# ugadiarov-la-phystech-edu/OCRL

Hardware: AMD Instinct MI355X
Metric: images/sec (node) SLATE pretrain 128x128, 6 slots, 3 iters (higher is better)
Workload: dtype f32

## Files before the change

ocrl_amd/_lib.py:

```python
import ctypes
import os
from ctypes import c_void_p

from . import _abi

_HERE = os.path.dirname(os.path.abspath(__file__))
LIB_PATH = os.environ.get("OCRL_HIP_LIB") or os.path.join(_HERE, "libocrl_hip.so")
HEADER_PATH = os.path.join(_HERE, os.pardir, "include", "ocrl_hip.h")
DQN_HEADER_PATH = os.path.join(_HERE, os.pardir, "include", "ocrl_hip_dqn.h")
ROLLOUT_HEADER_PATH = os.path.join(_HERE, os.pardir, "include", "ocrl_hip_rollout.h")
REPLAY_HEADER_PATH = os.path.join(_HERE, os.pardir, "include", "ocrl_hip_replay.h")
C51_HEADER_PATH = os.path.join(_HERE, os.pardir, "include", "ocrl_hip_c51.h")
NOISY_HEADER_PATH = os.path.join(_HERE, os.pardir, "include", "ocrl_hip_noisy.h")
CLASSIFIER_HEADER_PATH = os.path.join(_HERE, os.pardir, "include", "ocrl_hip_classifier.h")
IODINE_HEADER_PATH = os.path.join(_HERE, os.pardir, "include", "ocrl_hip_iodine.h")
QR_HEADER_PATH = os.path.join(_HERE, os.pardir, "include", "ocrl_hip_qr.h")
SLATE_KERNELS_HEADER_PATH = os.path.join(_HERE, os.pardir, "include", "ocrl_hip_slate_kernels.h")
_lib = None

if not os.path.exists(HEADER_PATH):
    raise RuntimeError(f"{HEADER_PATH} is missing: ocrl_amd derives its binding of libocrl_hip.so from the header and runs from the source tree.")
with open(HEADER_PATH) as _f:
    ABI = _abi.read(_f.read())
CONSTANTS = ABI.consts
SlateConfig, IodineConfig, GemmDesc, ConvDesc, ConvWgradDesc, XattnDesc, AcnetDesc, SpriteEnvDesc, ScenesDesc, FlatSegment = (
    ABI.structs["ocrl_" + n] for n in ("slate_config", "iodine_config", "gemm_desc", "conv_desc", "conv_wgrad_desc", "xattn_desc", "acnet_desc",
                                       "sprite_env_desc", "scenes_desc", "flat_segment"))
FLAT_MAX_SEGMENTS = CONSTANTS["OCRL_FLAT_MAX_SEGMENTS"]
if not os.path.exists(DQN_HEADER_PATH):
    raise RuntimeError(f"{DQN_HEADER_PATH} is missing: ocrl_amd derives its binding of libocrl_hip.so from the header and runs from the source tree.")
with open(DQN_HEADER_PATH) as _f:
    ABI_DQN = _abi.read(_f.read())
QnetDesc = ABI_DQN.structs["ocrl_qnet_desc"]
QNET_MAX_LAYERS = len(QnetDesc().dims)
if not os.path.exists(ROLLOUT_HEADER_PATH):
    raise RuntimeError(f"{ROLLOUT_HEADER_PATH} is missing: ocrl_amd derives its binding of libocrl_hip.so from the header and runs from the source tree.")
with open(ROLLOUT_HEADER_PATH) as _f:
    ABI_ROLLOUT = _abi.read(_f.read())
if not os.path.exists(REPLAY_HEADER_PATH):
    raise RuntimeError(f"{REPLAY_HEADER_PATH} is missing: ocrl_amd derives its binding of libocrl_hip.so from the header and runs from the source tree.")
with open(REPLAY_HEADER_PATH) as _f:
    ABI_REPLAY = _abi.read(_f.read())
if not os.path.exists(C51_HEADER_PATH):
    raise RuntimeError(f"{C51_HEADER_PATH} is missing: ocrl_amd derives its binding of libocrl_hip.so from the header and runs from the source tree.")
with open(C51_HEADER_PATH) as _f:
    ABI_C51 = _abi.read(_f.read())
C51Desc = ABI_C51.structs["ocrl_c51_desc"]
if not os.path.exists(NOISY_HEADER_PATH):
    raise RuntimeError(f"{NOISY_HEADER_PATH} is missing: ocrl_amd derives its binding of libocrl_hip.so from the header and runs from the source tree.")
with open(NOISY_HEADER_PATH) as _f:
    ABI_NOISY = _abi.read(_f.read())
NoisyDesc = ABI_NOISY.structs["ocrl_noisy_desc"]
NOISY_MAX_LAYERS = len(NoisyDesc().out)
if not os.path.exists(CLASSIFIER_HEADER_PATH):
    raise RuntimeError(f"{CLASSIFIER_HEADER_PATH} is missing: ocrl_amd derives its binding of libocrl_hip.so from the header and runs from the source tree.")
with open(CLASSIFIER_HEADER_PATH) as _f:
    ABI_CLASSIFIER = _abi.read(_f.read())
if not os.path.exists(IODINE_HEADER_PATH):
    raise RuntimeError(f"{IODINE_HEADER_PATH} is missing: ocrl_amd derives its binding of libocrl_hip.so from the header and runs from the source tree.")
with open(IODINE_HEADER_PATH) as _f:
    ABI_IODINE = _abi.read(_f.read())
if not os.path.exists(QR_HEADER_PATH):
    raise RuntimeError(f"{QR_HEADER_PATH} is missing: ocrl_amd derives its binding of libocrl_hip.so from the header and runs from the source tree.")
with open(QR_HEADER_PATH) as _f:
    ABI_QR = _abi.read(_f.read())
QrDesc = ABI_QR.structs["ocrl_qr_desc"]
if not os.path.exists(SLATE_KERNELS_HEADER_PATH):
    raise RuntimeError(f"{SLATE_KERNELS_HEADER_PATH} is missing: ocrl_amd derives its binding of libocrl_hip.so from the header and runs from the source tree.")
with open(SLATE_KERNELS_HEADER_PATH) as _f:
    ABI_SLATE_KERNELS = _abi.read(_f.read())


def flat_segments(segs):
    addr = lambda a: a.value if isinstance(a, c_void_p) else a
    return (FlatSegment * len(segs))(*[FlatSegment(addr(p), addr(g), addr(s0), addr(s1), int(n)) for p, g, s0, s1, n in segs])


def acnet_desc(B, F, A, dims, acts):
    d = AcnetDesc(B=B, F=F, A=A)
    for t in range(3):
        if len(dims[t]) > CONSTANTS["OCRL_ACNET_MAX_LAYERS"]:
            raise ValueError(f"ocrl_amd: at most {CONSTANTS['OCRL_ACNET_MAX_LAYERS']} layers per trunk (got {len(dims[t])})")
        d.n[t] = len(dims[t])
        for l, (w, a) in enumerate(zip(dims[t], acts[t])):
            d.dims[t][l], d.acts[t][l] = int(w), int(a)
    return d


def qnet_desc(B, F, A, dims, acts):
    if len(dims) > QNET_MAX_LAYERS or len(acts) != len(dims):
        raise ValueError(f"ocrl_amd: at most {QNET_MAX_LAYERS} hidden layers, one activation code each (got {len(dims)}, {len(acts)})")
    d = QnetDesc(B=B, F=F, A=A, n=len(dims))
    for l, (w, a) in enumerate(zip(dims, acts)):
        d.dims[l], d.acts[l] = int(w), int(a)
    return d


def c51_desc(B, F, A, Z, dims, acts, dueling=False):
    if len(dims) > len(C51Desc().dims) or len(acts) != len(dims):
        raise ValueError(f"ocrl_amd: at most {len(C51Desc().dims)} hidden layers, one activation code each (got {len(dims)}, {len(acts)})")
    d = C51Desc(B=B, F=F, A=A, Z=Z, n=len(dims), dueling=int(bool(dueling)))
    for l, (w, a) in enumerate(zip(dims, acts)):
        d.dims[l], d.acts[l] = int(w), int(a)
    return d


def qr_desc(B, F, A, N, dims, acts, dueling=False):
    if len(dims) > len(QrDesc().dims) or len(acts) != len(dims):
        raise ValueError(f"ocrl_amd: at most {len(QrDesc().dims)} hidden layers, one activation code each (got {len(dims)}, {len(acts)})")
    d = QrDesc(B=B, F=F, A=A, N=N, n=len(dims), dueling=int(bool(dueling)))
    for l, (w, a) in enumerate(zip(dims, acts)):
        d.dims[l], d.acts[l] = int(w), int(a)
    return d


def noisy_desc(layers):
    layers = list(layers)
    if not 1 <= len(layers) <= NOISY_MAX_LAYERS:
        raise ValueError(f"ocrl_amd: 1 .. {NOISY_MAX_LAYERS} noisy layers (got {len(layers)})")
    d = NoisyDesc(n_layers=len(layers))
    for l, (i, o) in enumerate(layers):
        getattr(d, "in")[l], d.out[l] = int(i), int(o)
    return d


def gemm_desc(**kw):
    d = GemmDesc(batch=1, batch_inner=1, splitk=1, alpha=1.0, x_scale=1.0, e_scale=1.0, force_sb=-1)
    for k, v in kw.items():
        setattr(d, k, v)
    return d


def conv_desc(**kw):
    d = ConvDesc()
    for k, v in kw.items():
        setattr(d, k, v)
    return d


def conv_wgrad_desc(**kw):
    d = ConvWgradDesc()
    for k, v in kw.items():
        setattr(d, k, v)
    return d


def lib():
    global _lib
    if _lib is not None:
        return _lib
    if not os.path.exists(LIB_PATH):
        raise RuntimeError(
            f"{LIB_PATH} is missing: build it with `python -c 'import __graft_entry__ as g; g.build()'` "
            "(make -C ocrl_amd/csrc).  ocrl_amd has no CPU fallback.")
    import torch
    L = ctypes.CDLL(LIB_PATH)
    for abi in (ABI, ABI_DQN, ABI_ROLLOUT, ABI_REPLAY, ABI_C51, ABI_NOISY, ABI_CLASSIFIER, ABI_IODINE, ABI_QR, ABI_SLATE_KERNELS):
        for name, (restype, argtypes) in abi.functions.items():
            f = getattr(L, name)
            f.argtypes = argtypes
            if restype is not ctypes.c_int:
                f.restype = restype
    for name, cls in {**ABI.structs, **ABI_DQN.structs, **ABI_C51.structs, **ABI_NOISY.structs, **ABI_QR.structs}.items():
        if name + "_size" in {**ABI.functions, **ABI_DQN.functions, **ABI_C51.functions, **ABI_NOISY.functions, **ABI_QR.functions} and getattr(L, name + "_size")() != ctypes.sizeof(cls):
            raise RuntimeError(f"libocrl_hip.so: {name} is {getattr(L, name + '_size')()} bytes, this binding's {cls.__name__} {ctypes.sizeof(cls)}")
    if L.ocrl_abi_version() != CONSTANTS["OCRL_ABI_VERSION"]:
        raise RuntimeError(f"libocrl_hip.so ABI version mismatch: the library is {L.ocrl_abi_version()}, include/ocrl_hip.h {CONSTANTS['OCRL_ABI_VERSION']}")
    _lib = L
    return L


def check(rc):
    if rc:
        raise RuntimeError("ocrl_hip: " + lib().ocrl_last_error().decode())


def ptr(t):
    return None if t is None else ctypes.c_void_p(t.data_ptr())


def ptrs(ts):
    return (ctypes.c_void_p * len(ts))(*[t.data_ptr() if t is not None else None for t in ts])


def stream(device=None):
    import torch
    return ctypes.c_void_p(torch.cuda.current_stream(device).cuda_stream)
```

ocrl_amd/csrc/elementwise.hip:

```cpp
#include "common.h"
#include "kernels.h"
#include "layernorm16.h"

#define TINYF 1.17549435e-38f

__device__ inline float block_sum(float v, float* red) {
    v = wave_sum(v);
    const int w = threadIdx.x >> 6, nw = blockDim.x >> 6;
    __syncthreads();
    if ((threadIdx.x & 63) == 0) red[w] = v;
    __syncthreads();
    float s = 0.f;
    for (int i = 0; i < nw; ++i) s += red[i];
    return s;
}
__device__ inline float block_max(float v, float* red) {
    v = wave_max(v);
    const int w = threadIdx.x >> 6, nw = blockDim.x >> 6;
    __syncthreads();
    if ((threadIdx.x & 63) == 0) red[w] = v;
    __syncthreads();
    float s = red[0];
    for (int i = 1; i < nw; ++i) s = fmaxf(s, red[i]);
    return s;
}

__global__ void nchw_to_nhwc8_kernel(const float* __restrict__ in, float* __restrict__ out, int B, int C, int H, int W) {
    const long long n = (long long)B * H * W;
    const long long i = (long long)blockIdx.x * blockDim.x + threadIdx.x;
    if (i >= n) return;
    const long long hw = (long long)H * W;
    const long long b = i / hw, r = i % hw;
    float v[8];
#pragma unroll
    for (int c = 0; c < 8; ++c) v[c] = c < C ? in[(b * C + c) * hw + r] : 0.f;
    float4* o = reinterpret_cast<float4*>(out + i * 8);
    o[0] = make_float4(v[0], v[1], v[2], v[3]);
    o[1] = make_float4(v[4], v[5], v[6], v[7]);
}

__global__ void patchify4_kernel(const float* __restrict__ in, float* __restrict__ out, int B, int C, int S) {
    const int E = S / 4;
    const long long n = (long long)B * E * E * C * 4;
    const long long i = (long long)blockIdx.x * blockDim.x + threadIdx.x;
    if (i >= n) return;
    const int ky = i & 3;
    const int c = (i >> 2) % C;
    const long long row = (i >> 2) / C;
    const int ex = row % E, ey = (row / E) % E;
    const long long b = row / ((long long)E * E);
    const float4 v = *reinterpret_cast<const float4*>(in + ((b * C + c) * S + (ey * 4 + ky)) * S + ex * 4);
    *reinterpret_cast<float4*>(out + row * (C * 16) + c * 16 + ky * 4) = v;
}

__global__ void pixel_shuffle_kernel(const float* __restrict__ in, float* __restrict__ out, int B, int h, int w, int Cout, int forward,
                                     const float* __restrict__ mask) {
    const long long n = (long long)B * h * w * Cout;
    const long long i = (long long)blockIdx.x * blockDim.x + threadIdx.x;
    if (i >= n) return;
    const int c = i % Cout;
    long long r = i / Cout;
    const int x = r % w; r /= w;
    const int y = r % h;
    const long long b = r / h;
    const long long u = i * 4;
    const long long s00 = ((b * 2 * h + 2 * y) * (2 * w) + 2 * x) * Cout + c;
    const long long s01 = s00 + Cout, s10 = s00 + (long long)2 * w * Cout, s11 = s10 + Cout;
    if (forward) {
        const float4 v = *reinterpret_cast<const float4*>(in + u);
        out[s00] = v.x; out[s01] = v.y; out[s10] = v.z; out[s11] = v.w;
    } else {
        float4 v = make_float4(in[s00], in[s01], in[s10], in[s11]);
        if (mask) {
            const float4 m = *reinterpret_cast<const float4*>(mask + u);
            v.x = m.x > 0.f ? v.x : 0.f; v.y = m.y > 0.f ? v.y : 0.f; v.z = m.z > 0.f ? v.z : 0.f; v.w = m.w > 0.f ? v.w : 0.f;
        }
        *reinterpret_cast<float4*>(out + u) = v;
    }
}

template <int NPL>
__global__ void layernorm_fwd_kernel(const float* __restrict__ x, const float* __restrict__ g, const float* __restrict__ bta,
                                     float* __restrict__ y, float* __restrict__ mean, float* __restrict__ rstd, long long R) {
    constexpr int F = 64 * NPL;
    const int lane = threadIdx.x & 63;
    const long long row = (long long)blockIdx.x * (blockDim.x >> 6) + (threadIdx.x >> 6);
    if (row >= R) return;
    float v[NPL];
    float s = 0.f;
#pragma unroll
    for (int i = 0; i < NPL; ++i) { v[i] = x[row * F + i * 64 + lane]; s += v[i]; }
    const float mu = wave_sum(s) * (1.0f / F);
    float q = 0.f;
#pragma unroll
    for (int i = 0; i < NPL; ++i) { const float d = v[i] - mu; q += d * d; }
    const float rs = rsqrtf(wave_sum(q) * (1.0f / F) + 1e-5f);
#pragma unroll
    for (int i = 0; i < NPL; ++i) {
        const int c = i * 64 + lane;
        y[row * F + c] = (v[i] - mu) * rs * g[c] + bta[c];
    }
    if (lane == 0) {
        if (mean) mean[row] = mu;
        if (rstd) rstd[row] = rs;
    }
}

template <int NPL>
__global__ void layernorm_bwd_kernel(const float* __restrict__ dy, const float* __restrict__ x, const float* __restrict__ mean,
                                     const float* __restrict__ rstd, const float* __restrict__ g, float* __restrict__ dx,
                                     float* __restrict__ part, long long R, int accumulate) {
    constexpr int F = 64 * NPL;
    __shared__ float red[4][2 * F];
    const int lane = threadIdx.x & 63, wv = threadIdx.x >> 6;
    float dg[NPL], db[NPL], gg[NPL];
#pragma unroll
    for (int i = 0; i < NPL; ++i) { dg[i] = 0.f; db[i] = 0.f; gg[i] = g[i * 64 + lane]; }
    for (long long row = (long long)blockIdx.x * 4 + wv; row < R; row += (long long)gridDim.x * 4) {
        const float mu = mean[row], rs = rstd[row];
        float xh[NPL], d[NPL];
        float s1 = 0.f, s2 = 0.f;
#pragma unroll
        for (int i = 0; i < NPL; ++i) {
            const int c = i * 64 + lane;
            xh[i] = (x[row * F + c] - mu) * rs;
            const float dyv = dy[row * F + c];
            dg[i] += dyv * xh[i];
            db[i] += dyv;
            d[i] = dyv * gg[i];
            s1 += d[i];
            s2 += d[i] * xh[i];
        }
        s1 = wave_sum(s1) * (1.0f / F);
        s2 = wave_sum(s2) * (1.0f / F);
#pragma unroll
        for (int i = 0; i < NPL; ++i) {
            const int c = i * 64 + lane;
            const float v = rs * (d[i] - s1 - xh[i] * s2);
            dx[row * F + c] = accumulate ? dx[row * F + c] + v : v;
        }
    }
#pragma unroll
    for (int i = 0; i < NPL; ++i) { red[wv][i * 64 + lane] = dg[i]; red[wv][F + i * 64 + lane] = db[i]; }
    __syncthreads();
    for (int c = threadIdx.x; c < 2 * F; c += blockDim.x)
        part[(size_t)blockIdx.x * 2 * F + c] = red[0][c] + red[1][c] + red[2][c] + red[3][c];
}

template <int NV, int NP>
__global__ __launch_bounds__(256) void layernorm16_fwd_kernel(const float* __restrict__ x, const float* __restrict__ g, const float* __restrict__ bta,
                                                              float* __restrict__ y, float* __restrict__ mean, float* __restrict__ rstd, long long R) {
    constexpr int F = 64 * NV;
    const int lane = threadIdx.x & 63, wv = threadIdx.x >> 6, c4 = lane & 15, rsub = lane >> 4;
    const long long row0 = ((long long)blockIdx.x * 4 + wv) * (4 * NP) + rsub;
    float4 v[NP][NV];
#pragma unroll
    for (int i = 0; i < NP; ++i)
#pragma unroll
        for (int k = 0; k < NV; ++k) {
            const long long row = row0 + 4 * i;
            v[i][k] = row < R ? *reinterpret_cast<const float4*>(x + row * F + (k * 16 + c4) * 4) : make_float4(0.f, 0.f, 0.f, 0.f);
        }
    float4 gg[NV], bb[NV];
#pragma unroll
    for (int k = 0; k < NV; ++k) { gg[k] = *reinterpret_cast<const float4*>(g + (k * 16 + c4) * 4); bb[k] = *reinterpret_cast<const float4*>(bta + (k * 16 + c4) * 4); }
#pragma unroll
    for (int i = 0; i < NP; ++i) {
        const long long row = row0 + 4 * i;
        float mu, rs;
        layernorm16_row_fwd<NV>(v[i], mu, rs);
        if (row < R) {
#pragma unroll
            for (int k = 0; k < NV; ++k) *reinterpret_cast<float4*>(y + row * F + (k * 16 + c4) * 4) = layernorm16_affine(v[i][k], rs, gg[k], bb[k]);
            if (c4 == 0) {
                if (mean) mean[row] = mu;
                if (rstd) rstd[row] = rs;
            }
        }
    }
}
template <int NV, int NP>
__global__ __launch_bounds__(256) void layernorm16_bwd_kernel(const float* __restrict__ dy, const float* __restrict__ x, const float* __restrict__ mean,
                                                              const float* __restrict__ rstd, const float* __restrict__ g, float* __restrict__ dx,
                                                              float* __restrict__ part, long long R, int accumulate) {
    constexpr int F = 64 * NV;
    __shared__ float4 red[2][16][16 * NV];
    const int lane = threadIdx.x & 63, wv = threadIdx.x >> 6, c4 = lane & 15, rsub = lane >> 4;
    float4 gg[NV], dg[NV], db[NV];
#pragma unroll
    for (int k = 0; k < NV; ++k) { gg[k] = *reinterpret_cast<const float4*>(g + (k * 16 + c4) * 4); dg[k] = make_float4(0.f, 0.f, 0.f, 0.f); db[k] = dg[k]; }
    for (long long grp = blockIdx.x; grp * (16 * NP) < R; grp += gridDim.x) {
        const long long row0 = (grp * 4 + wv) * (4 * NP) + rsub;
        float4 xv[NP][NV], yv[NP][NV];
        float mu[NP], rs[NP];
#pragma unroll
        for (int i = 0; i < NP; ++i) {
            const long long row = row0 + 4 * i;
            const bool ok = row < R;
#pragma unroll
            for (int k = 0; k < NV; ++k) {
                xv[i][k] = ok ? *reinterpret_cast<const float4*>(x + row * F + (k * 16 + c4) * 4) : make_float4(0.f, 0.f, 0.f, 0.f);
                yv[i][k] = ok ? *reinterpret_cast<const float4*>(dy + row * F + (k * 16 + c4) * 4) : make_float4(0.f, 0.f, 0.f, 0.f);
            }
            mu[i] = ok ? mean[row] : 0.f;
            rs[i] = ok ? rstd[row] : 0.f;
        }
#pragma unroll
        for (int i = 0; i < NP; ++i) {
            const long long row = row0 + 4 * i;
            const Ln16Bwd<NV> r = layernorm16_row_bwd<NV>(xv[i], yv[i], mu[i], rs[i], gg, dg, db);
            if (row < R) {
#pragma unroll
                for (int k = 0; k < NV; ++k) {
                    float4 o = layernorm16_row_dx(r, rs[i], k);
                    float* dp = dx + row * F + (k * 16 + c4) * 4;
                    if (accumulate) { const float4 a = *reinterpret_cast<const float4*>(dp); o.x += a.x; o.y += a.y; o.z += a.z; o.w += a.w; }
                    *reinterpret_cast<float4*>(dp) = o;
                }
            }
        }
    }
#pragma unroll
    for (int k = 0; k < NV; ++k) { red[0][wv * 4 + rsub][k * 16 + c4] = dg[k]; red[1][wv * 4 + rsub][k * 16 + c4] = db[k]; }
    __syncthreads();
    if (threadIdx.x < 32 * NV) {
        const int which = threadIdx.x / (16 * NV), c = threadIdx.x % (16 * NV);
        float4 a = red[which][0][c];
#pragma unroll
        for (int k = 1; k < 16; ++k) { const float4 t = red[which][k][c]; a.x += t.x; a.y += t.y; a.z += t.z; a.w += t.w; }
        *reinterpret_cast<float4*>(part + (size_t)blockIdx.x * (2 * F) + which * F + c * 4) = a;
    }
}

__global__ void colsum_kernel(const float* __restrict__ X, long long ld, float* __restrict__ part, long long R, int F, long long rows_per_chunk) {
    __shared__ float red[4][64];
    const int col = blockIdx.x * 64 + (threadIdx.x & 63), rl = threadIdx.x >> 6;
    const long long r0 = (long long)blockIdx.y * rows_per_chunk;
    const long long r1 = min(R, r0 + rows_per_chunk);
    float s = 0.f;
    if (col < F)
        for (long long r = r0 + rl; r < r1; r += 4) s += X[r * ld + col];
    red[rl][threadIdx.x & 63] = s;
    __syncthreads();
    if (rl == 0 && col < F) part[(size_t)blockIdx.y * F + col] = red[0][threadIdx.x] + red[1][threadIdx.x] + red[2][threadIdx.x] + red[3][threadIdx.x];
}
__global__ __launch_bounds__(256) void colsum4_kernel(const float* __restrict__ X, long long ld, float* __restrict__ part, long long R, int F,
                                                      long long rows_per_chunk) {
    __shared__ float4 red[256];
    const int F4 = F >> 2, RL = 256 / F4;
    const int c4 = threadIdx.x % F4, rl = threadIdx.x / F4;
    const long long r0 = (long long)blockIdx.x * rows_per_chunk;
    const long long r1 = min(R, r0 + rows_per_chunk);
    float4 s0 = make_float4(0.f, 0.f, 0.f, 0.f), s1 = s0, s2 = s0, s3 = s0;
    if (rl < RL) {
        const float* base = X + (size_t)c4 * 4;
        long long r = r0 + rl;
        for (; r + 3 * RL < r1; r += 4 * RL) {
            const float4 a = *reinterpret_cast<const float4*>(base + r * ld), b = *reinterpret_cast<const float4*>(base + (r + RL) * ld);
            const float4 c = *reinterpret_cast<const float4*>(base + (r + 2 * RL) * ld), d = *reinterpret_cast<const float4*>(base + (r + 3 * RL) * ld);
            s0.x += a.x; s0.y += a.y; s0.z += a.z; s0.w += a.w;
            s1.x += b.x; s1.y += b.y; s1.z += b.z; s1.w += b.w;
            s2.x += c.x; s2.y += c.y; s2.z += c.z; s2.w += c.w;
            s3.x += d.x; s3.y += d.y; s3.z += d.z; s3.w += d.w;
        }
        for (; r < r1; r += RL) {
            const float4 a = *reinterpret_cast<const float4*>(base + r * ld);
            s0.x += a.x; s0.y += a.y; s0.z += a.z; s0.w += a.w;
        }
    }
    red[threadIdx.x] = make_float4(s0.x + s1.x + s2.x + s3.x, s0.y + s1.y + s2.y + s3.y, s0.z + s1.z + s2.z + s3.z, s0.w + s1.w + s2.w + s3.w);
    __syncthreads();
    if (threadIdx.x < F4) {
        float4 t = red[threadIdx.x];
        for (int k = 1; k < RL; ++k) { const float4 v = red[k * F4 + threadIdx.x]; t.x += v.x; t.y += v.y; t.z += v.z; t.w += v.w; }
        *reinterpret_cast<float4*>(part + (size_t)blockIdx.x * F + threadIdx.x * 4) = t;
    }
}
__global__ __launch_bounds__(256) void colsum_final_kernel(const float* __restrict__ part, float* __restrict__ out, int nchunk, int F, int accumulate, float scale) {
    __shared__ float red[16][16];
    const int cl = threadIdx.x & 15, rl = threadIdx.x >> 4;
    const int c = blockIdx.x * 16 + cl;
    float s0 = 0.f, s1 = 0.f;
    if (c < F) {
        int k = rl;
        for (; k + 16 < nchunk; k += 32) { s0 += part[(size_t)k * F + c]; s1 += part[(size_t)(k + 16) * F + c]; }
        if (k < nchunk) s0 += part[(size_t)k * F + c];
    }
    red[rl][cl] = s0 + s1;
    __syncthreads();
    if (rl == 0 && c < F) {
        float t = 0.f;
#pragma unroll
        for (int k = 0; k < 16; ++k) t += red[k][cl];
        t *= scale;
        out[c] = accumulate ? out[c] + t : t;
    }
}

__global__ void reduce_partials_kernel(const float* __restrict__ part, int n, float* __restrict__ out, float scale, int accumulate) {
    __shared__ float red[4];
    float s = 0.f;
    for (int i = threadIdx.x; i < n; i += blockDim.x) s += part[i];
    s = block_sum(s, red);
    if (threadIdx.x == 0) out[0] = (accumulate ? out[0] : 0.f) + s * scale;
}

__global__ void mse_kernel(const float* __restrict__ obs, const float* __restrict__ recon, float* __restrict__ drecon,
                           float* __restrict__ part, int B, int C, int H, int W, float inv_b) {
    __shared__ float red[4];
    const long long n = (long long)B * H * W, hw = (long long)H * W;
    float s = 0.f;
    for (long long i = (long long)blockIdx.x * blockDim.x + threadIdx.x; i < n; i += (long long)gridDim.x * blockDim.x) {
        const long long b = i / hw, r = i % hw;
        const float4 rc = *reinterpret_cast<const float4*>(recon + i * 4);
        const float rv[4] = {rc.x, rc.y, rc.z, rc.w};
        float d[4] = {0.f, 0.f, 0.f, 0.f};
        for (int c = 0; c < C; ++c) {
            const float e = rv[c] - obs[(b * C + c) * hw + r];
            s += e * e;
            d[c] = 2.f * e * inv_b;
        }
        if (drecon) *reinterpret_cast<float4*>(drecon + i * 4) = make_float4(d[0], d[1], d[2], d[3]);
    }
    s = block_sum(s, red);
    if (threadIdx.x == 0) part[blockIdx.x] = s;
}

#define GS_MAXPT 16
template <int NPT>
__global__ __launch_bounds__(256) void gumbel_softmax_kernel(const float* __restrict__ raw, const float* __restrict__ e1,
                                                             const float* __restrict__ e2, float* __restrict__ z,
                                                             int* __restrict__ tokens, int V, float inv_tau,
                                                             unsigned long long seed, float* __restrict__ zst) {
    __shared__ float red[4];
    __shared__ float redv[4];
    __shared__ int redi[4];
    const long long row = blockIdx.x;
    const float* r = raw + row * V;
    const int npt = NPT ? NPT : V / 256;
    float x[GS_MAXPT];
    float mx = -INFINITY;
#pragma unroll
    for (int i = 0; i < GS_MAXPT; ++i)
        if (i < npt) { x[i] = r[i * 256 + threadIdx.x]; mx = fmaxf(mx, x[i]); }
    mx = block_max(mx, red);
    float s = 0.f;
#pragma unroll
    for (int i = 0; i < GS_MAXPT; ++i)
        if (i < npt) s += __expf(x[i] - mx);
    s = block_sum(s, red);
    const float lse = mx + __logf(s);
    float u[GS_MAXPT];
    float best = -INFINITY;
    int besti = 0;
    float m2 = -INFINITY;
#pragma unroll
    for (int i = 0; i < GS_MAXPT; ++i)
        if (i < npt) {
            const int v = i * 256 + threadIdx.x;
            const float lp = x[i] - lse;
            float ea, eb;
            if (e1) { ea = e1[row * V + v]; eb = e2[row * V + v]; }
            else {
                const uint64_t idx = (uint64_t)row * V + v;
                const uint2 ba = rng_bits4(seed, SITE_GUMBEL_Z, idx);
                ea = -__logf(u01_24(ba.x));
                eb = -__logf(u01_24(ba.y));
            }
            const float g1 = -__logf(ea + TINYF), g2 = -__logf(eb + TINYF);
            u[i] = (lp + g1) * inv_tau;
            m2 = fmaxf(m2, u[i]);
            const float h = (lp + g2) * inv_tau;
            if (h > best) { best = h; besti = v; }
        }
    m2 = block_max(m2, red);
    float s2 = 0.f;
#pragma unroll
    for (int i = 0; i < GS_MAXPT; ++i)
        if (i < npt) { u[i] = __expf(u[i] - m2); s2 += u[i]; }
    s2 = block_sum(s2, red);
    const float inv = 1.0f / s2;
#pragma unroll
    for (int i = 0; i < GS_MAXPT; ++i)
        if (i < npt) z[row * V + i * 256 + threadIdx.x] = u[i] * inv;
    if (zst) {
        float b1 = -1.f;
        int b1i = 0;
#pragma unroll
        for (int i = 0; i < GS_MAXPT; ++i)
            if (i < npt && u[i] > b1) { b1 = u[i]; b1i = i * 256 + threadIdx.x; }
        wave_argmax(b1, b1i);
        __shared__ float hv[4];
        __shared__ int hi[4];
        if ((threadIdx.x & 63) == 0) { hv[threadIdx.x >> 6] = b1; hi[threadIdx.x >> 6] = b1i; }
        __syncthreads();
        for (int k = 0; k < 4; ++k)
            if (hv[k] > b1 || (hv[k] == b1 && hi[k] < b1i)) { b1 = hv[k]; b1i = hi[k]; }
#pragma unroll
        for (int i = 0; i < GS_MAXPT; ++i)
            if (i < npt) {
                const int v = i * 256 + threadIdx.x;
                const float ys = u[i] * inv;
                zst[row * V + v] = ((v == b1i ? 1.f : 0.f) - ys) + ys;
            }
    }
    wave_argmax(best, besti);
    const int w = threadIdx.x >> 6;
    if ((threadIdx.x & 63) == 0) { redv[w] = best; redi[w] = besti; }
    __syncthreads();
    if (threadIdx.x == 0) {
        for (int k = 1; k < 4; ++k)
            if (redv[k] > best || (redv[k] == best && redi[k] < besti)) { best = redv[k]; besti = redi[k]; }
        tokens[row] = besti;
    }
}

template <int NPT>
__global__ __launch_bounds__(256) void softmax_bwd_rows_kernel(const float* __restrict__ z, float* __restrict__ d, int V, float scale) {
    __shared__ float red[4];
    const long long row = blockIdx.x;
    const int npt = NPT ? NPT : V / 256;
    float zz[GS_MAXPT], dd[GS_MAXPT];
    float s = 0.f;
#pragma unroll
    for (int i = 0; i < GS_MAXPT; ++i)
        if (i < npt) {
            zz[i] = z[row * V + i * 256 + threadIdx.x];
            dd[i] = d[row * V + i * 256 + threadIdx.x];
            s += zz[i] * dd[i];
        }
    s = block_sum(s, red);
#pragma unroll
    for (int i = 0; i < GS_MAXPT; ++i)
        if (i < npt) d[row * V + i * 256 + threadIdx.x] = zz[i] * (dd[i] - s) * scale;
}

struct CdfArgs { const float* scores; int V; float tau; unsigned long long seed; };
__device__ __forceinline__ float wave_incl_scan(float v, int lane) {
#pragma unroll
    for (int o = 1; o < 64; o <<= 1) {
        const float t = __shfl_up(v, o, 64);
        if (lane >= o) v += t;
    }
    return v;
}
__global__ __launch_bounds__(1024) void softmax_stat_combine_kernel(const float* __restrict__ stat, int nseg, long long R, float* __restrict__ lse,
                                                                    const float* __restrict__ hstat, const int* __restrict__ hidx,
                                                                    int* __restrict__ tokens, const float* __restrict__ pred, int ldp,
                                                                    const int* __restrict__ tok, float* __restrict__ part, CdfArgs cdf) {
// ... 351 lines not shown
}
__global__ void store_u64_kernel(unsigned long long* dst, unsigned long long v) { *dst = v; }
__global__ void slot_init_kernel(const float* __restrict__ mu, const float* __restrict__ logsig, const float* __restrict__ noise,
                                 float* __restrict__ slots0, long long n, int D, unsigned long long seed, const unsigned long long* __restrict__ seed_dev) {
    const long long i = (long long)blockIdx.x * blockDim.x + threadIdx.x;
    if (i >= n) return;
    if (seed_dev) seed = *seed_dev;
    const int c = i % D;
    slots0[i] = mu[c] + __expf(logsig[c]) * slot_eps(noise, i, seed);
}
__global__ __launch_bounds__(1024) void slot_init_bwd_kernel(const float* __restrict__ d, const float* __restrict__ logsig, const float* __restrict__ noise,
                                                             float* __restrict__ dmu, float* __restrict__ dlogsig, int R, int D, unsigned long long seed) {
    __shared__ float ra[16][64], rb[16][64];
    const int cl = threadIdx.x & 63, rl = threadIdx.x >> 6;
    const int c = blockIdx.x * 64 + cl;
    float a = 0.f, b = 0.f;
    if (c < D)
        for (int r = rl; r < R; r += 16) {
            const float g = d[(size_t)r * D + c];
            a += g;
            b += g * slot_eps(noise, (long long)r * D + c, seed);
        }
    ra[rl][cl] = a; rb[rl][cl] = b;
    __syncthreads();
    if (rl == 0 && c < D) {
        float sa = 0.f, sb = 0.f;
#pragma unroll
        for (int k = 0; k < 16; ++k) { sa += ra[k][cl]; sb += rb[k][cl]; }
        dmu[c] = sa;
        dlogsig[c] = sb * __expf(logsig[c]);
    }
}
__global__ void copy_kernel(const float* __restrict__ src, float* __restrict__ dst, long long n) {
    const long long i = (long long)blockIdx.x * blockDim.x + threadIdx.x;
    if (i < n) dst[i] = src[i];
}

__global__ __launch_bounds__(256) void argmax_pos_kernel(const float* __restrict__ pred, int* __restrict__ tokens, int T, int V, int t, int dense_rows) {
    __shared__ float rv[4];
    __shared__ int ri[4];
    const long long row = (long long)blockIdx.x * T + t;
    const float* r = pred + (dense_rows ? (long long)blockIdx.x : row) * V;
    float best = -INFINITY;
    int bi = 0;
    for (int v = threadIdx.x; v < V; v += 256) { const float x = r[v]; if (x > best) { best = x; bi = v; } }
    wave_argmax(best, bi);
    if ((threadIdx.x & 63) == 0) { rv[threadIdx.x >> 6] = best; ri[threadIdx.x >> 6] = bi; }
    __syncthreads();
    if (threadIdx.x == 0) {
        for (int k = 1; k < 4; ++k) if (rv[k] > best || (rv[k] == best && ri[k] < bi)) { best = rv[k]; bi = ri[k]; }
        tokens[row] = bi;
    }
}
__global__ void embed_step_kernel(const int* __restrict__ tokens, const float* __restrict__ dict, const float* __restrict__ bos,
                                  const float* __restrict__ pe, float* __restrict__ out, int B, int T, int d, int t) {
    const int i = blockIdx.x * blockDim.x + threadIdx.x;
    if (i >= B * d) return;
    const int b = i / d, c = i - b * d;
    const float* src = t == 0 ? bos : dict + (size_t)tokens[b * T + t - 1] * d;
    out[i] = src[c] + pe[(size_t)t * d + c];
}
__global__ __launch_bounds__(256) void decode_attn_kernel(const float* __restrict__ qkv, float* __restrict__ out, int T, int t, int d, int h, int ld) {
    extern __shared__ float sm[];
    const int dh = d / h, nk = t + 1, tid = threadIdx.x;
    float* sc = sm;
    float* qs = sc + ((T + 3) & ~3);
    float* red = qs + 64;
    const int b = blockIdx.x / h, hd = blockIdx.x % h;
    const float* base = qkv + (size_t)b * T * ld + hd * dh;
    const float scale = rsqrtf((float)dh);
    if (tid < dh) qs[tid] = base[(size_t)t * ld + tid] * scale;
    __syncthreads();
    float mx = -INFINITY;
    for (int j = tid; j < nk; j += 256) {
        const float* kr = base + (size_t)j * ld + d;
        float a = 0.f;
        for (int c = 0; c < dh; c += 4) {
            const float4 kv = *reinterpret_cast<const float4*>(kr + c);
            a += qs[c] * kv.x + qs[c + 1] * kv.y + qs[c + 2] * kv.z + qs[c + 3] * kv.w;
        }
        sc[j] = a;
        mx = fmaxf(mx, a);
    }
    red[tid] = mx;
    __syncthreads();
    block_tree_max<256>(red);
    mx = red[0];
    __syncthreads();
    float sum = 0.f;
    for (int j = tid; j < nk; j += 256) { const float e = __expf(sc[j] - mx); sc[j] = e; sum += e; }
    red[tid] = sum;
    __syncthreads();
    block_tree_sum<256>(red);
    const float inv = 1.0f / red[0];
    __syncthreads();
    const int nsl = 256 / dh, c = tid % dh, sl = tid / dh;
    float acc = 0.f;
    if (sl < nsl)
        for (int j = sl; j < nk; j += nsl) acc += sc[j] * base[(size_t)j * ld + 2 * d + c];
    red[tid] = sl < nsl ? acc : 0.f;
    __syncthreads();
    if (tid < dh) {
        float a = 0.f;
        for (int k = 0; k < nsl; ++k) a += red[k * dh + tid];
        out[(size_t)b * d + hd * dh + tid] = a * inv;
    }
}

__global__ void onehot_kernel(const int* __restrict__ tokens, float* __restrict__ z, long long n, int V) {
    const long long i = (long long)blockIdx.x * blockDim.x + threadIdx.x;
    if (i >= n) return;
    z[i] = (int)(i % V) == tokens[i / V] ? 1.f : 0.f;
}

int nchw_to_nhwc8_launch(const float* in, float* out, int B, int C, int H, int W, hipStream_t st) {
    OCRL_REQUIRE(C <= 8, "nchw_to_nhwc8: C must be <= 8");
    const long long n = (long long)B * H * W;
    hipLaunchKernelGGL(nchw_to_nhwc8_kernel, GRID1D(n), 0, st, in, out, B, C, H, W);
    OCRL_CHECK_LAUNCH("nchw_to_nhwc8");
    return 0;
}
int patchify4_launch(const float* in, float* out, int B, int C, int S, hipStream_t st) {
    OCRL_REQUIRE(S % 4 == 0, "patchify4: S %% 4 != 0");
    const long long n = (long long)B * (S / 4) * (S / 4) * C * 4;
    hipLaunchKernelGGL(patchify4_kernel, GRID1D(n), 0, st, in, out, B, C, S);
    OCRL_CHECK_LAUNCH("patchify4");
    return 0;
}
int pixel_shuffle_launch(const float* in, float* out, int B, int h, int w, int Cout, int forward, const float* mask, hipStream_t st) {
    const long long n = (long long)B * h * w * Cout;
    hipLaunchKernelGGL(pixel_shuffle_kernel, GRID1D(n), 0, st, in, out, B, h, w, Cout, forward, mask);
    OCRL_CHECK_LAUNCH("pixel_shuffle");
    return 0;
}
int layernorm_fwd_launch(const float* x, const float* g, const float* b, float* y, float* mean, float* rstd, long long R, int F, hipStream_t st) {
    OCRL_REQUIRE(F % 64 == 0 && F >= 64 && F <= 256, "layernorm: F must be 64..256, multiple of 64 (got %d)", F);
    dim3 grid(cdiv(R, 4)), blk(256);
    const bool al16 = aligned16(x, y, g, b);
    switch (F / 64) {
        case 1:
            if (al16) hipLaunchKernelGGL((layernorm16_fwd_kernel<1, 4>), dim3((unsigned)cdiv(R, 64)), blk, 0, st, x, g, b, y, mean, rstd, R);
            else hipLaunchKernelGGL(layernorm_fwd_kernel<1>, grid, blk, 0, st, x, g, b, y, mean, rstd, R);
            break;
        case 2: hipLaunchKernelGGL(layernorm_fwd_kernel<2>, grid, blk, 0, st, x, g, b, y, mean, rstd, R); break;
        case 3:
            if (al16) hipLaunchKernelGGL((layernorm16_fwd_kernel<3, 2>), dim3((unsigned)cdiv(R, 32)), blk, 0, st, x, g, b, y, mean, rstd, R);
            else hipLaunchKernelGGL(layernorm_fwd_kernel<3>, grid, blk, 0, st, x, g, b, y, mean, rstd, R);
            break;
        default: hipLaunchKernelGGL(layernorm_fwd_kernel<4>, grid, blk, 0, st, x, g, b, y, mean, rstd, R); break;
    }
    OCRL_CHECK_LAUNCH("layernorm_fwd");
    return 0;
}
int colsum_launch(const float* X, long long ld, float* out, long long R, int F, int accumulate, float scale, float* ws, size_t ws_floats, hipStream_t st) {
    if (F % 4 == 0 && ld % 4 == 0 && F <= 1024 && F >= 4 && (((uintptr_t)X) & 15) == 0 && R >= 1024) {
        long long nchunk = 2048;
        if (nchunk > R / 8) nchunk = R / 8;
        if ((size_t)nchunk * F > ws_floats) nchunk = (long long)(ws_floats / F);
        if (nchunk >= 16) {
            const long long rpc = (R + nchunk - 1) / nchunk;
            nchunk = (R + rpc - 1) / rpc;
            hipLaunchKernelGGL(colsum4_kernel, dim3((unsigned)nchunk), dim3(256), 0, st, X, ld, ws, R, F, rpc);
            OCRL_CHECK_LAUNCH("colsum4");
            hipLaunchKernelGGL(colsum_final_kernel, dim3(cdiv(F, 16)), dim3(256), 0, st, ws, out, (int)nchunk, F, accumulate, scale);
            OCRL_CHECK_LAUNCH("colsum_final");
            return 0;
        }
    }
    const int cb = cdiv(F, 64);
    long long nchunk = 1024 / cb;
    if (nchunk < 1) nchunk = 1;
    if (nchunk > (R + 63) / 64) nchunk = (R + 63) / 64;
    if (nchunk < 1) nchunk = 1;
    OCRL_REQUIRE((size_t)nchunk * F <= ws_floats, "colsum: workspace too small (%lld x %d)", nchunk, F);
    const long long rpc = (R + nchunk - 1) / nchunk;
    hipLaunchKernelGGL(colsum_kernel, dim3(cb, (int)nchunk), dim3(256), 0, st, X, ld, ws, R, F, rpc);
    OCRL_CHECK_LAUNCH("colsum");
    hipLaunchKernelGGL(colsum_final_kernel, dim3(cdiv(F, 16)), dim3(256), 0, st, ws, out, (int)nchunk, F, accumulate, scale);
    OCRL_CHECK_LAUNCH("colsum_final");
    return 0;
}
int layernorm_bwd_launch(const float* dy, const float* x, const float* mean, const float* rstd, const float* g, float* dx,
                         float* dgb, long long R, int F, int accumulate_dx, int accumulate_dgb, float* ws, size_t ws_floats, hipStream_t st) {
    OCRL_REQUIRE(F % 64 == 0 && F >= 64 && F <= 256, "layernorm bwd: F must be 64..256, multiple of 64 (got %d)", F);
    int nblk = (int)((R + 3) / 4);
    if (nblk > 2048) nblk = 2048;
    while (nblk > 64 && (size_t)nblk * 2 * F * 2 + (size_t)8 * 2 * F > ws_floats) nblk /= 2;
    const size_t need = (size_t)nblk * 2 * F;
    OCRL_REQUIRE(need + (size_t)8 * 2 * F <= ws_floats, "layernorm bwd: workspace too small");
    dim3 grid(nblk), blk(256);
    const bool al16 = aligned16(x, dy, dx, g, ws);
    switch (F / 64) {
        case 1:
            if (al16) hipLaunchKernelGGL((layernorm16_bwd_kernel<1, 4>), grid, blk, 0, st, dy, x, mean, rstd, g, dx, ws, R, accumulate_dx);
            else hipLaunchKernelGGL(layernorm_bwd_kernel<1>, grid, blk, 0, st, dy, x, mean, rstd, g, dx, ws, R, accumulate_dx);
            break;
        case 2: hipLaunchKernelGGL(layernorm_bwd_kernel<2>, grid, blk, 0, st, dy, x, mean, rstd, g, dx, ws, R, accumulate_dx); break;
        case 3:
            if (al16) hipLaunchKernelGGL((layernorm16_bwd_kernel<3, 2>), grid, blk, 0, st, dy, x, mean, rstd, g, dx, ws, R, accumulate_dx);
            else hipLaunchKernelGGL(layernorm_bwd_kernel<3>, grid, blk, 0, st, dy, x, mean, rstd, g, dx, ws, R, accumulate_dx);
            break;
        default: hipLaunchKernelGGL(layernorm_bwd_kernel<4>, grid, blk, 0, st, dy, x, mean, rstd, g, dx, ws, R, accumulate_dx); break;
    }
    OCRL_CHECK_LAUNCH("layernorm_bwd");
    return colsum_launch(ws, 2 * F, dgb, nblk, 2 * F, accumulate_dgb, 1.f, ws + need, ws_floats - need, st);
}
int reduce_partials_launch(const float* part, int n, float* out, float scale, int accumulate, hipStream_t st) {
    hipLaunchKernelGGL(reduce_partials_kernel, dim3(1), dim3(256), 0, st, part, n, out, scale, accumulate);
    OCRL_CHECK_LAUNCH("reduce_partials");
    return 0;
}
int mse_launch(const float* obs, const float* recon, float* drecon, float* out, int B, int C, int H, int W, float* ws, size_t ws_floats, hipStream_t st) {
    OCRL_REQUIRE(C <= 4, "mse: C must be <= 4");
    const int nblk = 1024;
    OCRL_REQUIRE(ws_floats >= (size_t)nblk, "mse: workspace too small");
    hipLaunchKernelGGL(mse_kernel, dim3(nblk), dim3(256), 0, st, obs, recon, drecon, ws, B, C, H, W, 1.0f / B);
    OCRL_CHECK_LAUNCH("mse");
    return reduce_partials_launch(ws, nblk, out, 1.0f / B, 0, st);
}
int gumbel_softmax_launch(const float* raw, const float* e1, const float* e2, float* z, int* tokens, long long R, int V, float tau,
                          unsigned long long seed, hipStream_t st, float* zst) {
    OCRL_REQUIRE(V % 256 == 0 && V <= 256 * GS_MAXPT, "gumbel_softmax: V must be a multiple of 256, <= %d", 256 * GS_MAXPT);
    OCRL_REQUIRE((e1 == nullptr) == (e2 == nullptr), "gumbel_softmax: give both noise tensors or none");
    switch (V / 256) {
        case 16: hipLaunchKernelGGL(gumbel_softmax_kernel<16>, dim3((unsigned)R), dim3(256), 0, st, raw, e1, e2, z, tokens, V, 1.0f / tau, seed, zst); break;
        case 8: hipLaunchKernelGGL(gumbel_softmax_kernel<8>, dim3((unsigned)R), dim3(256), 0, st, raw, e1, e2, z, tokens, V, 1.0f / tau, seed, zst); break;
        default: hipLaunchKernelGGL(gumbel_softmax_kernel<0>, dim3((unsigned)R), dim3(256), 0, st, raw, e1, e2, z, tokens, V, 1.0f / tau, seed, zst); break;
    }
    OCRL_CHECK_LAUNCH("gumbel_softmax");
    return 0;
}
int softmax_bwd_rows_launch(const float* z, float* d, long long R, int V, float scale, hipStream_t st) {
    OCRL_REQUIRE(V % 256 == 0 && V <= 256 * GS_MAXPT, "softmax_bwd_rows: V must be a multiple of 256, <= %d", 256 * GS_MAXPT);
    if (V == 4096) hipLaunchKernelGGL(softmax_bwd_rows_kernel<16>, dim3((unsigned)R), dim3(256), 0, st, z, d, V, scale);
    else hipLaunchKernelGGL(softmax_bwd_rows_kernel<0>, dim3((unsigned)R), dim3(256), 0, st, z, d, V, scale);
    OCRL_CHECK_LAUNCH("softmax_bwd_rows");
    return 0;
}
int softmax_stat_combine_launch(const float* stat, int nseg, long long R, float* lse, const float* hstat, const int* hidx, int* tokens,
                                const float* pred, int ldp, const int* tok, float* out, float scale, float* ws, size_t ws_floats, hipStream_t st,
                                const float* cdf_scores, int cdf_V, float cdf_tau, unsigned long long cdf_seed) {
    OCRL_REQUIRE(nseg >= 1 && nseg <= 64, "softmax_stat_combine: 1..64 segments (got %d)", nseg);
    const long long nblk = (R + 15) / 16;
    OCRL_REQUIRE(!pred || (tok && out && ws && ws_floats >= (size_t)nblk), "softmax_stat_combine: cross-entropy needs tokens, an output and %lld workspace floats", nblk);
    CdfArgs cdf;
    cdf.scores = cdf_scores; cdf.V = cdf_V; cdf.tau = cdf_tau; cdf.seed = cdf_seed;
    OCRL_REQUIRE(!cdf_scores || (hstat && hidx && tokens && cdf_V > 0 && cdf_V <= nseg * 64), "softmax_stat_combine: inverse-CDF sampling arguments");
    hipLaunchKernelGGL(softmax_stat_combine_kernel, dim3((unsigned)nblk), dim3(1024), 0, st, stat, nseg, R, lse, hstat, hidx, tokens, pred, ldp, tok,
                       pred ? ws : nullptr, cdf);
    OCRL_CHECK_LAUNCH("softmax_stat_combine");
    if (pred) return reduce_partials_launch(ws, (int)nblk, out, scale, 0, st);
    return 0;
}
int exp_rows_launch(const float* y, const float* lse, float* z, long long R, int V, hipStream_t st) {
    OCRL_REQUIRE(V % 4 == 0, "exp_rows: V %% 4 != 0");
    const long long n4 = R * (V / 4);
    hipLaunchKernelGGL(exp_rows_kernel, dim3((unsigned)((n4 + 255) / 256)), dim3(256), 0, st, y, lse, z, n4, V / 4);
    OCRL_CHECK_LAUNCH("exp_rows");
    return 0;
}
int rowdot_bias64_launch(const float* g, const float* act, const float* bias, long long R, float* out, hipStream_t st) {
    OCRL_REQUIRE(((((uintptr_t)g) | ((uintptr_t)act) | ((uintptr_t)bias)) & 15) == 0, "rowdot: operands must be 16-byte aligned");
    hipLaunchKernelGGL(rowdot_bias64_kernel, dim3((unsigned)((R + 15) / 16)), dim3(256), 0, st, g, act, bias, R, out);
    OCRL_CHECK_LAUNCH("rowdot_bias64");
    return 0;
}
int embed_fwd_launch(const int* tokens, const float* dict, const float* bos, const float* pe, float* out, int B, int T, int d, float p,
                     unsigned long long seed, hipStream_t st) {
    OCRL_REQUIRE(d % 4 == 0, "embed: d %% 4 != 0");
    const long long n = (long long)B * T * (d / 4);
    hipLaunchKernelGGL(embed_fwd_kernel, dim3((unsigned)cdiv(n, 1024)), dim3(256), 0, st, tokens, dict, bos, pe, out, B, T, d, p, seed);
    OCRL_CHECK_LAUNCH("embed_fwd");
    return 0;
}
static size_t eb_align(size_t n) { return (n + 63) & ~(size_t)63; }
size_t embed_bwd_ws_floats(long long BT, int V, int d) {
    const size_t nchunk = (size_t)cdiv(BT, EB_CHUNK), nunit = (size_t)cdiv(BT, EB_UNIT);
    return eb_align(nchunk * (V + 1)) + 2 * eb_align((size_t)V + 2) + eb_align((size_t)BT) + eb_align(nunit * 2 * d);
}
int embed_bwd_launch(float* g, const int* tokens, float* ddict, int B, int T, int V, int d, float p, unsigned long long seed, float* ws,
                     size_t ws_floats, hipStream_t st) {
    const long long BT = (long long)B * T;
    OCRL_REQUIRE(d % 4 == 0 && d <= 1024 && V + 1 <= 16384 && BT < (1ll << 31), "embed_bwd: unsupported shape (d %d, vocabulary %d, %lld rows)", d, V, BT);
    OCRL_REQUIRE(ws && ws_floats >= embed_bwd_ws_floats(BT, V, d), "embed_bwd: scratch too small");
    const int nchunk = cdiv(BT, EB_CHUNK), nunit = cdiv(BT, EB_UNIT);
    int* hist = reinterpret_cast<int*>(ws);
    int* total = hist + eb_align((size_t)nchunk * (V + 1));
    int* base = total + eb_align((size_t)V + 2);
    int* perm = base + eb_align((size_t)V + 2);
    float* part = reinterpret_cast<float*>(perm + eb_align((size_t)BT));
    if (p > 0.f) {
        hipLaunchKernelGGL(embed_drop_bwd_kernel, GRID1D(BT * (d / 4)), 0, st, g, B, T, d, p, seed);
        OCRL_CHECK_LAUNCH("embed_drop_bwd");
    }
    hipLaunchKernelGGL(eb_hist_kernel, dim3(nchunk), dim3(256), (V + 1) * sizeof(int), st, tokens, hist, BT, T, V);
    hipLaunchKernelGGL(eb_scan_chunks_kernel, dim3(cdiv(V + 1, 256)), dim3(256), 0, st, hist, total, nchunk, V);
    hipLaunchKernelGGL(eb_base_kernel, dim3(1), dim3(1024), 0, st, total, base, V);
    hipLaunchKernelGGL(eb_place_kernel, dim3(nchunk), dim3(256), 0, st, tokens, hist, base, perm, BT, T, V);
    const int nthr = (d + 63) & ~63;
    hipLaunchKernelGGL(eb_segsum_kernel, dim3(nunit), dim3(nthr), 0, st, g, tokens, perm, base, total, ddict, part, BT, T, V, d);
    hipLaunchKernelGGL(eb_combine_kernel, dim3(V), dim3(nthr), 0, st, base, total, part, ddict, V, d);
    OCRL_CHECK_LAUNCH("embed_bwd");
    return 0;
}
int dropout_apply_launch(const float* x, float* y, long long n, float p, unsigned long long seed, unsigned site, hipStream_t st) {
    OCRL_REQUIRE(n % 4 == 0, "dropout_apply: n %% 4 != 0");
    hipLaunchKernelGGL(dropout_apply_kernel, GRID1D(n / 4), 0, st, x, y, n / 4, p, seed, site);
    OCRL_CHECK_LAUNCH("dropout_apply");
    return 0;
}
int dropout_mask_launch(float* y, long long n, float p, unsigned long long seed, unsigned site, hipStream_t st) {
    hipLaunchKernelGGL(dropout_mask_kernel, GRID1D(n), 0, st, y, n, p, seed, site);
    OCRL_CHECK_LAUNCH("dropout_mask");
    return 0;
}
__global__ void obs_u8_to_f32_kernel(const unsigned char* __restrict__ in, float* __restrict__ out, long long npix_total, long long HW, int C) {
    const long long i = (long long)blockIdx.x * blockDim.x + threadIdx.x;
    if (i >= npix_total) return;
    const long long b = i / HW, pix = i - b * HW;
    const unsigned char* src = in + i * C;
    float* dst = out + b * C * HW + pix;
    for (int c = 0; c < C; ++c) dst[c * HW] = (float)src[c] / 255.0f;
}
int obs_u8_to_f32_launch(const unsigned char* in, float* out, int B, int H, int W, int C, hipStream_t st) {
    const long long n = (long long)B * H * W;
    hipLaunchKernelGGL(obs_u8_to_f32_kernel, GRID1D(n), 0, st, in, out, n, (long long)H * W, C);
    OCRL_CHECK_LAUNCH("obs_u8_to_f32");
    return 0;
}
int fill_launch(float* x, long long n, float v, hipStream_t st) {
    hipLaunchKernelGGL(fill_kernel, GRID1D(n), 0, st, x, n, v);
    OCRL_CHECK_LAUNCH("fill");
    return 0;
}
int axpy_launch(const float* x, float* y, long long n, float a, hipStream_t st) {
    hipLaunchKernelGGL(axpy_kernel, GRID1D(n), 0, st, x, y, n, a);
    OCRL_CHECK_LAUNCH("axpy");
    return 0;
}
int posmap_launch(const float* Wpos, const float* bpos, float* out, int S, int C, hipStream_t st) {
    hipLaunchKernelGGL(posmap_kernel, GRID1D((long long)S * S * C), 0, st, Wpos, bpos, out, S, C);
    OCRL_CHECK_LAUNCH("posmap");
    return 0;
}
int posgrid_launch(float* out, int S, hipStream_t st) {
    hipLaunchKernelGGL(posgrid_kernel, GRID1D(S * S), 0, st, out, S);
    OCRL_CHECK_LAUNCH("posgrid");
    return 0;
}
int pad_cols_launch(const float* in, int ldi, float* out, int ldo, long long R, int C, int Cout, hipStream_t st) {
    hipLaunchKernelGGL(pad_cols_kernel, GRID1D(R * Cout), 0, st, in, ldi, out, ldo, R, C, Cout);
    OCRL_CHECK_LAUNCH("pad_cols");
    return 0;
}
int store_u64_launch(unsigned long long* dst, unsigned long long v, hipStream_t st) {
    hipLaunchKernelGGL(store_u64_kernel, dim3(1), dim3(1), 0, st, dst, v);
    OCRL_CHECK_LAUNCH("store_u64");
    return 0;
// ... 57 lines not shown
```

ocrl_amd/csrc/kernels.h:

```cpp
#pragma once
#include "common.h"
#include "../../include/ocrl_hip.h"

enum { PROF_CONV5 = 0, PROF_CONV_OTHER = 1, PROF_WGRAD = 2, PROF_GEMM = 3, PROF_SA_FWD = 4, PROF_SA_BWD = 5, PROF_ATTN_FWD = 6, PROF_ATTN_BWD = 7, PROF_NTAGS = 8 };
int prof_begin(int tag, hipStream_t st);
void prof_end(int idx, hipStream_t st);

struct GemmArgs {
    const float* A = nullptr;
    const float* B = nullptr;
    float* C = nullptr;
    int M = 0, N = 0, K = 0;
    int lda = 0, ldb = 0, ldc = 0;
    int akc = 1, bkc = 1;
    int batch = 1;
    int batch_inner = 1;
    long long sA = 0, sB = 0, sC = 0;
    long long sAi = 0, sBi = 0, sCi = 0;
    int splitk = 1;
    long long sCsplit = 0;
    float alpha = 1.f;
    const float* bias = nullptr;
    int relu = 0;
    float drop_p = 0.f;
// ... 60 lines not shown
    float p = 0.f; unsigned long long seed = 0; unsigned site = 0;
};
int pool_cls_attn_fwd_launch(const PoolClsArgs& a, hipStream_t st);
int pool_cls_attn_bwd_launch(const PoolClsArgs& a, hipStream_t st);
int pool_flash_launch(const float* qkv, float* O, float* lse, const float* dO, float* Dd, float* dqkv, int B, int S, int d, int h, float p,
                      unsigned long long seed, unsigned site, int backward, hipStream_t st);

int rn_pair_fwd_launch(const float* AB, const float* b1, float* h1, int B, int K, int g, hipStream_t st);
int rn_pair_bwd_launch(const float* dh1, float* dAB, int B, int K, int g, hipStream_t st);
int rn_pairsum_fwd_launch(const float* gL, float* y, int B, int P, int g, hipStream_t st);
int rn_pairsum_bwd_launch(const float* dy, const float* gL, float* dgL, int B, int P, int g, hipStream_t st);

struct NcMap { long long sN = 0, sG = 0, sC = 0, sH = 0, sW = 0; };
struct NcFwdArgs {
    const float* X = nullptr; NcMap x;
    float* Y = nullptr; float* Y2 = nullptr; NcMap y;
    const float* w[OCRL_NATURECNN_MAX_GROUPS] = {}; const float* bias[OCRL_NATURECNN_MAX_GROUPS] = {};
    int B = 0, G = 1, cin = 0, cout = 0, H = 0, W = 0, OH = 0, OW = 0, ks = 0, stride = 0;
    int pad = 0;
};
struct NcBwdArgs {
    const float* X = nullptr; NcMap x;
    const float* dY = nullptr; NcMap dy;
    float* dX = nullptr;
    float* part = nullptr;
    int slabs = 1, slab_rows = 0;
    const float* w[OCRL_NATURECNN_MAX_GROUPS] = {};
    int B = 0, G = 1, cin = 0, cout = 0, H = 0, W = 0, OH = 0, OW = 0, ks = 0, stride = 0;
    int pad = 0;
    long long dw_tiles = 0, dx_tiles = 0; int dw_blocks = 0;
};
struct NcReduceLayer { const float* part = nullptr; int slabs = 0, G = 0, cout = 0, K = 0; long long n = 0; };
struct NcReduceArgs {
    NcReduceLayer L[OCRL_NATURECNN_MAX_CONVS];
    float* dw[OCRL_NATURECNN_MAX_CONVS][OCRL_NATURECNN_MAX_GROUPS] = {};
    float* db[OCRL_NATURECNN_MAX_CONVS][OCRL_NATURECNN_MAX_GROUPS] = {};
    int nlayers = 0;
};
int nc_conv_fwd_launch(const NcFwdArgs& a, hipStream_t st);
int nc_conv_bwd_launch(NcBwdArgs a, hipStream_t st);
int nc_dw_reduce_launch(const NcReduceArgs& a, hipStream_t st);
int nc_relu_mask_launch(const float* d, const float* act, float* out, long long n, hipStream_t st);

struct PcGeom {
    int OH = 0, OW = 0, OWT = 0;
    int NG = 0, nchunk = 0;
    size_t wp_floats = 0;
    long long units = 0; int slab_units = 0, slabs = 0; size_t part_floats = 0;
    int passes = 0, nbg = 0, Dp = 0; size_t wd_floats = 0;
    int HB = 0, WB = 0, WT = 0; long long dx_units = 0; int upw = 0;
};
PcGeom pc_geom(int B, int H, int W, int D);
struct PcFwdArgs {
    const float* X = nullptr; const float* Wp = nullptr; const float* bias = nullptr; float* Y = nullptr;
    int B = 0, H = 0, W = 0, D = 0, OH = 0, OW = 0, OWT = 0, nchunk = 0, NG = 0;
};
struct PcDwArgs {
    const float* X = nullptr; const float* dY = nullptr; float* part = nullptr; float* partb = nullptr;
    int B = 0, H = 0, W = 0, D = 0, OH = 0, OW = 0, OWT = 0, nchunk = 0, slab_units = 0;
    long long units = 0;
};
struct PcDxArgs {
    const float* dY = nullptr; const float* Wd = nullptr; float* dX = nullptr;
    int H = 0, W = 0, D = 0, OH = 0, OW = 0, HB = 0, WT = 0, Dp = 0, passes = 0, upw = 0;
    long long units = 0, groups = 0;
};
int pc_conv1_fwd_launch(const float* X, const float* w, const float* bias, float* Wp, float* Y, int B, int H, int W, int D, hipStream_t st);
int pc_conv1_dw_launch(const float* X, const float* dY, float* part, int B, int H, int W, int D, hipStream_t st);
int pc_conv1_dw_reduce_launch(const float* part, float* dw, float* db, int B, int H, int W, int D, hipStream_t st);
int pc_conv1_dx_launch(const float* dY, const float* w, float* Wd, float* dX, int B, int H, int W, int D, hipStream_t st);

#define PROBE_MAX_SLOTS 12
#define PROBE_MAX_PROPS 8
#define PROBE_MAX_WIDTH 256
struct ProbeSchema { int P; int t[PROBE_MAX_PROPS], a[PROBE_MAX_PROPS], b[PROBE_MAX_PROPS], kind[PROBE_MAX_PROPS]; };
int probe_schema_check(const ProbeSchema& sc, int T, int O);
int probe_match_check(int B, int K, int N, int T, int O);
int probe_match_launch(const float* out, int ld_row, long long ld_img, const float* y, const float* dloss, float* cost, int* col, float* part,
                       float* metrics, float* dout, int B, int K, int N, int T, int O, const ProbeSchema& sc, hipStream_t st);
int probe_leaky_fwd_launch(float* x, long long n, float slope, hipStream_t st);
int probe_leaky_bwd_launch(float* dx, const float* h, long long n, float slope, hipStream_t st);

int vae_permute_launch(const float* src, float* dst, long long R, int C, int HW, int rows, int pack, hipStream_t st);
int vae_pad_rows_launch(const float* src, float* dst, int rows, int rows_pad, int K, hipStream_t st);
int vae_kl_fwd_launch(const float* ml, const float* eps, float* latent, float* part, float* rep, int B, int L, hipStream_t st);
int vae_loss_launch(const float* part, float* metrics, int B, float kld_weight, hipStream_t st);
int vae_kl_bwd_launch(const float* ml, const float* eps, const float* dlat, const float* drep, const float* dloss, float* dml, int B, int L,
                      float kld_weight, hipStream_t st);
int vae_scale_launch(const float* x, float* y, const float* g, long long n, hipStream_t st);
int vae_recon_nchw_launch(const float* r4, float* out, int B, int C, int HW, hipStream_t st);

#define MAE_MAX_PATCHES 1024
int mae_rank_launch(const float* noise, int* restore, int* keep, float* mask, int* restore_out, float* mask_out, int B, int L, int len_keep,
                    hipStream_t st);
int mae_patch_gather_launch(const float* obs, const int* ids, float* out, int B, int n, int S, int p, hipStream_t st);
int mae_tokens_fwd_launch(const float* embed, const float* cls, const float* pos, const int* ids, float* x0, int B, int n, int D, hipStream_t st);
int mae_tokens_bwd_launch(const float* dx0, float* dembed, float* dcls, int B, int n, int D, hipStream_t st);
int mae_unshuffle_fwd_launch(const float* e, const float* mtok, const float* dpos, const int* restore, float* xd, int B, int L, int len_keep, int Dd,
                             hipStream_t st);
int mae_unshuffle_bwd_launch(const float* dxd, const int* keep, const float* mask, float* de, float* dmtok, float* part, int B, int L, int len_keep,
                             int Dd, hipStream_t st);
int mae_gelu_fwd_launch(const float* pre, float* y, long long n, hipStream_t st);
int mae_gelu_bwd_launch(const float* dy, const float* pre, float* dpre, long long n, hipStream_t st);
int mae_ln_fwd_launch(const float* x, const float* g, const float* b, float* y, float* mean, float* rstd, long long R, int F, float eps, hipStream_t st);
int mae_ln_chunks(long long R);
int mae_ln_bwd_launch(const float* dy, const float* x, const float* mean, const float* rstd, const float* g, const float* resid, float* dx, float* dg,
                      float* db, float* part, long long R, int F, hipStream_t st);
int mae_loss_launch(const float* pred, const float* obs, const float* mask, const float* dloss, float* part, float* loss, float* dpred, int B, int L,
                    int len_keep, int S, int p, hipStream_t st);

struct ConvArgs {
    const float* X = nullptr;
    const float* Wp = nullptr;
    float* Y = nullptr;
    int B = 0, H = 0, W = 0;
    const float* bias = nullptr;
    int relu = 0;
    const float* posmap = nullptr;
    const float* mask = nullptr;
    int mask_elu = 0;
};
size_t conv_x3_pack_floats(int KS = 5);
int conv_pack_x3_launch(const float* W, float* fwd3, float* bwd3, hipStream_t st, int KS = 5);
int conv_x3_launch(const ConvArgs& a, const float* pack3, hipStream_t st, int KS = 5);
struct WgradArgs;
int conv_wgrad_x3_stage(const WgradArgs& a, int nchunk, hipStream_t st, int KS = 5);
struct WgradArgs {
    const float* X = nullptr;
    const float* dY = nullptr;
    float* part = nullptr;
    int B = 0, H = 0, W = 0;
    float* bpart = nullptr;
};
int conv_fwd_launch(const ConvArgs& a, int KS, int CIN, int COUT, hipStream_t st, int low_latency = 0);
int conv_wgrad_launch(const WgradArgs& a, int KS, int CIN, int COUT, int cin_real, float* dW, float* db, int accumulate, hipStream_t st, int x3 = -1);
int conv_wgrad_slabs(int B, int H, int W, int KS, int CIN);
size_t conv_wgrad_ws_floats(int B, int H, int W, int KS, int CIN, bool with_db = true);
int conv_pack_launch(const float* W, float* fwd, float* bwd, int KS, int CIN, int COUT, int cin_real, hipStream_t st);

size_t conv_first_pack_floats();
int conv_first_pack_launch(const float* W, float* pack, hipStream_t st);
int conv_first_fwd_launch(const float* obs, const float* pack, const float* bias, float* Y, int B, int H, int W, int relu, hipStream_t st);
int conv_first_wgrad_workers(int B, int H, int W);
size_t conv_first_wgrad_ws_floats(int B, int H, int W);
int conv_first_wgrad_launch(const float* obs, const float* dY, float* ws, float* dW, float* db, int B, int H, int W, int accumulate, hipStream_t st);

int nchw_to_nhwc8_launch(const float* in, float* out, int B, int C, int H, int W, hipStream_t st);
int patchify4_launch(const float* in, float* out, int B, int C, int S, hipStream_t st);
int pixel_shuffle_launch(const float* in, float* out, int B, int h, int w, int Cout, int forward, const float* mask, hipStream_t st);
int layernorm_fwd_launch(const float* x, const float* g, const float* b, float* y, float* mean, float* rstd, long long R, int F, hipStream_t st);
int layernorm_bwd_launch(const float* dy, const float* x, const float* mean, const float* rstd, const float* g, float* dx,
                         float* dgb, long long R, int F, int accumulate_dx, int accumulate_dgb, float* ws, size_t ws_floats, hipStream_t st);
int colsum_launch(const float* X, long long ld, float* out, long long R, int F, int accumulate, float scale, float* ws, size_t ws_floats, hipStream_t st);

#define SA_INPUT_SLAB (2 * 4096 + 4 * 64)
void sa_input_plan(long long R, int max_wgs, int out[3]);
int sa_input_fwd_launch(const float* e4, const float* gamma, const float* beta, const float* W0, const float* b0, const float* W2, const float* b2,
                        float* mean, float* rstd, float* ln0, float* h1, float* x, long long R, int max_wgs, hipStream_t st);
int sa_input_bwd_launch(const float* dx, const float* h1, const float* e4, const float* mean, const float* rstd, const float* gamma, const float* beta,
                        const float* W0, const float* W2, float* de4, float* dW0, float* db0, float* dW2, float* db2, float* dgamma, float* dbeta,
                        long long R, int max_wgs, float* ws, size_t ws_floats, hipStream_t st);
int reduce_partials_launch(const float* part, int n, float* out, float scale, int accumulate, hipStream_t st);
int mse_launch(const float* obs, const float* recon, float* drecon, float* out, int B, int C, int H, int W, float* ws, size_t ws_floats, hipStream_t st);
int gumbel_softmax_launch(const float* raw, const float* e1, const float* e2, float* z, int* tokens, long long R, int V, float tau,
                          unsigned long long seed, hipStream_t st, float* zst = nullptr);
int softmax_bwd_rows_launch(const float* z, float* d, long long R, int V, float scale, hipStream_t st);
int softmax_stat_combine_launch(const float* stat, int nseg, long long R, float* lse, const float* hstat, const int* hidx, int* tokens,
                                const float* pred, int ldp, const int* tok, float* out, float scale, float* ws, size_t ws_floats, hipStream_t st,
                                const float* cdf_scores = nullptr, int cdf_V = 0, float cdf_tau = 1.f, unsigned long long cdf_seed = 0);
int exp_rows_launch(const float* y, const float* lse, float* z, long long R, int V, hipStream_t st);
int rowdot_bias64_launch(const float* g, const float* act, const float* bias, long long R, float* out, hipStream_t st);
int embed_fwd_launch(const int* tokens, const float* dict, const float* bos, const float* pe, float* out, int B, int T, int d, float p,
                     unsigned long long seed, hipStream_t st);
size_t embed_bwd_ws_floats(long long BT, int V, int d);
int embed_bwd_launch(float* g, const int* tokens, float* ddict, int B, int T, int V, int d, float p, unsigned long long seed, float* ws,
                     size_t ws_floats, hipStream_t st);
int dropout_apply_launch(const float* x, float* y, long long n, float p, unsigned long long seed, unsigned site, hipStream_t st);
int dropout_mask_launch(float* y, long long n, float p, unsigned long long seed, unsigned site, hipStream_t st);
int obs_u8_to_f32_launch(const unsigned char* in, float* out, int B, int H, int W, int C, hipStream_t st);
int fill_launch(float* x, long long n, float v, hipStream_t st);
int axpy_launch(const float* x, float* y, long long n, float a, hipStream_t st);
int posmap_launch(const float* Wpos, const float* bpos, float* out, int S, int C, hipStream_t st);
int posgrid_launch(float* out, int S, hipStream_t st);
int im2col5_launch(const float* x8, float* col, long long npix, int H, int W, int C, int ldc, hipStream_t st);
int unpack5_launch(const float* dWp, float* dW, int C, int ldc, hipStream_t st);
int pad_cols_launch(const float* in, int ldi, float* out, int ldo, long long R, int C, int Cout, hipStream_t st);

struct XaPlan { bool supported = false; int KP = 0, NC = 0, NM = 0; size_t lds = 0; };
bool xattn_plan(int K, int d, int h, XaPlan* out);
bool xattn_supported(int K, int d, int h);
int xattn_kp(int K, int h);
struct XaFoldHost {
    const float* mem = nullptr;
    const float* Wq[8]; const float* Wk[8]; const float* Wv[8]; const float* Wo[8];
    float* ck[8]; float* cv[8];
    float* Ab[8]; float* AbT[8]; float* Vo[8]; float* VoT[8];
    int B = 0, K = 0, d = 0, h = 0, nblk = 0;
};
int xattn_fold_fwd_launch(const XaFoldHost& f, hipStream_t st);
struct XaHost {
    const float* x = nullptr;
    const float* resid = nullptr;
    float* y = nullptr;
    float* P = nullptr;
    const float *Ab = nullptr, *AbT = nullptr, *Vo = nullptr, *VoT = nullptr;
    const float* gd = nullptr;
    float *Pd = nullptr, *dS = nullptr;
    int B = 0, T = 0, K = 0, d = 0, h = 0;
    float p = 0.f; unsigned long long seed = 0; unsigned site_p = 0, site_o = 0;
};
int xattn_launch(const XaHost& h, int backward, hipStream_t st);
struct XaFoldBwdHost {
    const float *Pd = nullptr, *dS = nullptr;
    const float *gd = nullptr, *x = nullptr;
    const float *Wq = nullptr, *Wo = nullptr;
    const float *ck = nullptr, *cv = nullptr;
    float *dVo = nullptr, *dAb = nullptr;
    float *dck = nullptr, *dcv = nullptr;
    float *pq = nullptr, *po = nullptr;
    float *dWq = nullptr, *dWo = nullptr;
    float* ws = nullptr; size_t ws_floats = 0;
    int B = 0, T = 0, K = 0, d = 0, h = 0;
};
int xattn_fold_bwd_launch(const XaFoldBwdHost& f, hipStream_t st);
int cross_attn_fwd_launch(const float* Q, const float* Km, const float* Vm, float* O, float* P, int B, int T, int K, int d, int h, float p,
                          unsigned long long seed, unsigned site, hipStream_t st);
size_t cross_attn_bwd_ws_floats(int B, int T, int K, int d, int h);
int cross_attn_bwd_launch(const float* dO, const float* Q, const float* Km, const float* Vm, const float* P, float* dQ, float* dKm, float* dVm,
                          int B, int T, int K, int d, int h, float p, unsigned long long seed, unsigned site, float* part, size_t part_floats,
                          hipStream_t st);


struct SaWts {
    int ln_in_g, ln_in_b, ln_s_g, ln_s_b, ln_m_g, ln_m_b;
    int Wq, WqT, Wk, WkT, Wv, WvT, Wih, WihT, Whh, WhhT, bih, bhh, W0, W0T, b0, W2, W2T, b2;
    int total;
};
static inline SaWts sa_wts_layout(int C, int D, int H) {
    SaWts o; int a = 0;
    auto take = [&](int n) { int r = a; a += (n + 3) & ~3; return r; };
    o.ln_in_g = take(C); o.ln_in_b = take(C); o.ln_s_g = take(D); o.ln_s_b = take(D); o.ln_m_g = take(D); o.ln_m_b = take(D);
    o.Wq = take(D * D); o.WqT = take(D * D); o.Wk = take(D * C); o.WkT = take(C * D); o.Wv = take(D * C); o.WvT = take(C * D);
    o.Wih = take(3 * D * D); o.WihT = take(3 * D * D); o.Whh = take(3 * D * D); o.WhhT = take(3 * D * D);
    o.bih = take(3 * D); o.bhh = take(3 * D);
    o.W0 = take(H * D); o.W0T = take(H * D); o.b0 = take(H); o.W2 = take(D * H); o.W2T = take(D * H); o.b2 = take(D);
    o.total = a;
    return o;
}
struct SaSave { int sprev, sn, q, u, r, z, n, hn, sg, m, hid, qp, up, upn, csum, ld; };
static inline SaSave sa_save_layout(int C, int D, int H, int NH = 1) {
    SaSave o;
    o.sprev = 0; o.sn = D; o.q = 2 * D; o.u = 3 * D; o.r = 4 * D; o.z = 5 * D; o.n = 6 * D; o.hn = 7 * D; o.sg = 8 * D; o.m = 9 * D;
    o.hid = 10 * D; o.qp = 10 * D + H; o.up = o.qp + NH * C; o.upn = o.up + NH * C; o.csum = o.upn + NH * C; o.ld = o.csum + ((NH + 3) & ~3);
    return o;
}
struct SaGrad { int out, hid, gi, gh, u, q, qp, ld; };
static inline SaGrad sa_grad_layout(int C, int D, int H, int NH = 1) {
    SaGrad o;
    o.out = 0; o.hid = D; o.gi = D + H; o.gh = 4 * D + H; o.u = 7 * D + H; o.q = 8 * D + H; o.qp = 9 * D + H; o.ld = 9 * D + H + NH * C;
    return o;
}
struct SlotAttnArgs {
    int B = 0, N = 0, C = 64, K = 0, D = 0, H = 0, I = 0;
    int NH = 1;
    float eps = 1e-8f, scale = 1.f;
    const float* x = nullptr;
    const float* slots0 = nullptr;
    const float* wts = nullptr;
    float* slots = nullptr;
    float* attn = nullptr;
    float* attn_heads = nullptr;
    float* save = nullptr;
    const float* dslots = nullptr;
    float* dx = nullptr;
    float* dslots0 = nullptr;
    float* grows = nullptr;
    float* g_small = nullptr;
    float* xchg = nullptr;
    float* parts = nullptr;
    int phase = 0;
};
size_t sa_xchg_floats_host(int K, int D);
size_t sa_parts_floats_host(int B, int K);
struct SaPlan { int G, NB, KB, KS; size_t smem_fwd, smem_bwd; };
int sa_plan(int K, int D, int H, int NH, SaPlan* plan);
int slot_attn_launch(const SlotAttnArgs& a, int backward, hipStream_t st);

struct PackEntry { const float* src; int rows, cols, dst_off, transpose; };
int pack_launch(const PackEntry* entries_dev, int n_entries, int max_elems, float* dst, hipStream_t st);

int absmax_launch(const float* g, long long n, float* out, float* ws, size_t ws_floats, hipStream_t st);
int clip_adam_launch(float* p, const float* g, float* m, float* v, long long n, const float* norm, float clip, float lr, double b1,
                     double b2, double eps, int step, float gscale, hipStream_t st);
int clip_adam_tail_launch(float* p, const float* g, float* m, float* v, int n, const float* norm, float clip, float lr, double b1, double b2,
                          double eps, int step, float gscale, hipStream_t st);
int clip_rmsprop_launch(float* p, const float* g, float* sq, long long n, const float* norm, float clip, float lr, double alpha, double eps,
                        hipStream_t st);
int clip_rmsprop_tail_launch(float* p, const float* g, float* sq, int n, const float* norm, float clip, float lr, double alpha, double eps,
                             hipStream_t st);
constexpr int FLAT_MAX_SEG = 8, FLAT_SEG_BLOCKS = 1024;
struct FlatSegs {
    float* p[FLAT_MAX_SEG];
    const float* g[FLAT_MAX_SEG];
    float* s0[FLAT_MAX_SEG];
    float* s1[FLAT_MAX_SEG];
    long long n[FLAT_MAX_SEG];
// ... 82 lines not shown
```

ocrl_amd/csrc/slate_model.cpp:

```cpp
#include "slate_model.h"

#include "switches.h"

#include <math.h>
#include <stdarg.h>
#include <string.h>

static std::string fmt(const char* f, ...) {
    char buf[256];
    va_list ap;
    va_start(ap, f);
    vsnprintf(buf, sizeof buf, f, ap);
    va_end(ap);
    return buf;
}

SlateModel::SlateModel(const SlateConfig& c) : cfg(c) {
    S = c.obs_size; E = S / 4; T = E * E; N = S * S; V = c.vocab; d = c.d_model; C = c.cnn_hidden;
    K = c.num_slots; I = c.num_iters; D = c.slot_size; H = c.mlp_hidden; NB = c.num_blocks; NH = c.num_heads;
    DH = d / NH; Bmax = c.max_batch; SH = c.slot_heads > 0 ? c.slot_heads : 1;
    const int ch = c.obs_channels;
    add_param("_dvae._encoder.0.m.weight", {64, ch, 4, 4}, 0); add_param("_dvae._encoder.0.m.bias", {64}, 0);
    for (int i = 1; i < 7; ++i) { add_param(fmt("_dvae._encoder.%d.m.weight", i), {64, 64, 1, 1}, 0); add_param(fmt("_dvae._encoder.%d.m.bias", i), {64}, 0); }
    add_param("_dvae._encoder.7.weight", {V, 64, 1, 1}, 0); add_param("_dvae._encoder.7.bias", {V}, 0);
// ... 84 lines not shown
    for (const ParamInfo& q : params_)
        if (q.group == 1 && (q.name.rfind("_slotproj.", 0) == 0 || q.name.rfind("_dec.", 0) == 0) && q.offset < w.enc_grads_end) w.enc_grads_end = q.offset;
}

SlateModel::~SlateModel() {
    if (ev_fork_) (void)hipEventDestroy(ev_fork_);
    if (ev_join_) (void)hipEventDestroy(ev_join_);
    if (ev_tokens_) (void)hipEventDestroy(ev_tokens_);
    if (side_) (void)hipStreamDestroy(side_);
    for (auto& kv : enc_graphs_) if (kv.second.exec) (void)hipGraphExecDestroy(kv.second.exec);
    for (hipEvent_t e : ev_dw_) if (e) (void)hipEventDestroy(e);
    if (ev_join2_) (void)hipEventDestroy(ev_join2_);
    if (side2_) (void)hipStreamDestroy(side2_);
    if (cap_) (void)hipStreamDestroy(cap_);
}

void SlateModel::layout_workspace(bool commit) {
    begin_layout(commit);
    x3_of_.clear();
    const size_t B = Bmax, BT = B * T, BN = B * N, BK = B * K;
    metrics_ = carve("metrics", 64);
    scratch_floats_ = 0;
    {
        size_t need = conv_wgrad_ws_floats((int)(B * (cfg.use_bcdec ? K : 1)), S, S, 5, 64) + (size_t)512 * 2304 * 2;
        if (conv_first_wgrad_ws_floats((int)B, S, S) > need) need = conv_first_wgrad_ws_floats((int)B, S, S);
        size_t sk = (size_t)32 * V * d + (size_t)(1 << 20);
        if (sk > need) need = sk;
        size_t cs = (size_t)N * C * 8 + (size_t)T * d * 8 + (1 << 20);
        if (cs > need) need = cs;
        if (cfg.use_bcdec && bcast_l1_bwd_ws_floats((long long)BK, S, 5) > need) need = bcast_l1_bwd_ws_floats((long long)BK, S, 5);
        const size_t ca = cross_attn_bwd_ws_floats((int)B, T, K, d, NH), eb = embed_bwd_ws_floats((long long)B * T, V, d);
        if (ca > need) need = ca;
        if (eb > need) need = eb;
        scratch_floats_ = need + (1 << 20);
    }
    scratch_ = carve(nullptr, scratch_floats_);
    scratch2_ = cfg.use_bcdec ? scratch_ : carve(nullptr, scratch_floats_);
    obs8_ = first_direct() ? nullptr : carve("obs8", BN * 8);
    obs_keep_ = first_direct() ? carve(nullptr, BN * cfg.obs_channels) : nullptr;
    obs_stage_ = carve(nullptr, (B < 32 ? B : 32) * (size_t)cfg.obs_channels * N);
    seed_dev_ = reinterpret_cast<unsigned long long*>(carve(nullptr, 64));
    e1_ = carve("enc1", BN * 64); e2_ = carve("enc2", BN * 64); e3_ = carve("enc3", BN * 64); e4_ = carve("feats", BN * 64);
    posmap_ = carve(nullptr, (size_t)N * C); gridT_ = carve(nullptr, (size_t)N * 4);
    ln0_ = carve(nullptr, BN * 64); ln0_mean_ = carve(nullptr, BN); ln0_rstd_ = carve(nullptr, BN);
    h1_ = carve("sa_mlp_hidden", BN * 64); x_ = carve("sa_inputs", BN * 64);
    slots0_ = carve("slots0", BK * D); slot_noise_ = carve(nullptr, BK * D); slots_ = carve("slots", BK * D);
    attn_ = carve("attn", BN * K);
    attn_heads_ = SH > 1 ? carve(nullptr, sa_attn_heads_floats(B, N, K, SH)) : nullptr;
    const SaSizes sz = sa_sizes(B, K, C, D, H, I, SH);
    sa_save_ = carve("sa_save", sz.save);
    sa_grows_ = carve(nullptr, sz.grows);
    sa_wts_ = carve(nullptr, sz.wts);
    sa_small_ = carve(nullptr, sz.small);
    sa_xchg_ = carve(nullptr, sz.xchg);
    sa_parts_ = carve(nullptr, sz.parts);
    sa_pack_dev_ = reinterpret_cast<PackEntry*>(carve(nullptr, sz.table));
    for (int i = 0; i < 4; ++i) {
        const int cin = i == 0 ? 8 : 64;
        cw_fwd_[i] = carve(nullptr, (size_t)25 * cin * 64);
        cw_bwd_[i] = i == 0 ? nullptr : carve(nullptr, (size_t)25 * 64 * 64);
        if (conv_x3_ && i > 0) {
            float* f3 = carve(nullptr, conv_x3_pack_floats());
            float* b3 = carve(nullptr, conv_x3_pack_floats());
            if (ws_commit_) { x3_of_[cw_fwd_[i]] = f3; x3_of_[cw_bwd_[i]] = b3; }
        }
    }
    gslots_ = carve(nullptr, BK * D); gslots0_ = carve(nullptr, BK * D);
    gA_ = carve(nullptr, BN * 64); gB_ = carve(nullptr, BN * 64); gC_ = cfg.use_bcdec ? gA_ : carve(nullptr, BN * 64);
    gmap_ = carve(nullptr, (size_t)N * C);
    if (cfg.use_bcdec) {
        const size_t BKN = BK * (size_t)N;
        bc_Wc_ = carve(nullptr, 25 * 64 * 5 + 64); bc_W1r_ = carve(nullptr, (size_t)25 * 64 * D); bc_P1_ = carve(nullptr, (size_t)N * 64);
        bc_M_ = carve(nullptr, BK * 1600); bc_T_ = carve(nullptr, BK * 1600);
        bc_c1_ = carve("bc_c1", BKN * 64); bc_c2_ = carve("bc_c2", BKN * 64); bc_c3_ = carve("bc_c3", BKN * 64);
        bc_out4_ = carve(nullptr, BKN * 4); bc_dout4_ = carve(nullptr, BKN * 4);
        bc_gA_ = carve(nullptr, BKN * 64); bc_gB_ = carve(nullptr, BKN * 64);
        for (int i = 0; i < 2; ++i) {
            bc_pk_[i] = carve(nullptr, 25 * 64 * 64); bc_pkb_[i] = carve(nullptr, 25 * 64 * 64);
            if (conv_x3_ > 0) {
                float* f3 = carve(nullptr, conv_x3_pack_floats());
                float* b3 = carve(nullptr, conv_x3_pack_floats());
                if (ws_commit_) { x3_of_[bc_pk_[i]] = f3; x3_of_[bc_pkb_[i]] = b3; }
            }
        }
        bc_Wk4_ = carve(nullptr, 9 * 64 * 4); bc_Wb4_ = carve(nullptr, 9 * 64 * 4);
        bc_dW1r_ = carve(nullptr, (size_t)25 * 64 * D); bc_dWc_ = carve(nullptr, 25 * 64 * 5 + 64);
        bc_dT_ = carve(nullptr, BK * 1600); bc_dM_ = carve(nullptr, BK * 1600); bc_G1_ = carve(nullptr, (size_t)N * 64);
        recon_ = carve("recon", BN * 4);
    } else {
    patches_ = carve("patches", BT * 16 * cfg.obs_channels);
    for (int i = 0; i < 7; ++i) de_[i] = carve(fmt("dvae_enc%d", i).c_str(), BT * 64);
    zraw_ = carve("zraw", BT * V);
    z_ = carve("z", BT * V);
    zdec_ = cfg.hard ? carve("z_st", BT * V) : z_;
    tokens_ = reinterpret_cast<int*>(carve("tokens", BT));
    {
        const size_t nseg = (size_t)gemm_stat_segments(V);
        zstat_ = carve(nullptr, BT * nseg * 2); zhstat_ = carve(nullptr, BT * nseg); zhidx_ = reinterpret_cast<int*>(carve(nullptr, BT * nseg));
        zlse_ = carve("z_lse", BT); zdot_ = carve(nullptr, BT);
        cestat_ = carve(nullptr, BT * nseg * 2); celse_ = carve("ce_lse", BT); cepart_ = carve(nullptr, BT / 16 + 16);
    }
    dd0_ = carve("dvae_dec0", BT * 64); dd1_ = carve("dvae_dec1", BT * 64); dd2_ = carve("dvae_dec2", BT * 64); dd3_ = carve("dvae_dec3", BT * 64);
    dd4_ = carve("dvae_dec4", BT * 256); ps1_ = carve(nullptr, BT * 256);
    dd6_ = carve("dvae_dec6", BT * 256); dd7_ = carve("dvae_dec7", BT * 256); dd8_ = carve("dvae_dec8", BT * 256);
    dd9_ = carve("dvae_dec9", BT * 1024); ps2_ = carve(nullptr, BN * 64);
    recon_ = carve("recon", BN * 4); drecon_ = carve(nullptr, BN * 4);
    for (int i = 0; i < 2; ++i) {
        dw_fwd_[i] = carve(nullptr, 9 * 64 * 64); dw_bwd_[i] = carve(nullptr, 9 * 64 * 64);
        if (conv_x3_ > 0) {
            float* f3 = carve(nullptr, conv_x3_pack_floats(3));
            float* b3 = carve(nullptr, conv_x3_pack_floats(3));
            if (ws_commit_) { x3_of_[dw_fwd_[i]] = f3; x3_of_[dw_bwd_[i]] = b3; }
        }
    }
    w11p_ = carve(nullptr, 4 * 64);
    mem_ = carve("mem", BK * d); emb_ = carve("emb", BT * d);
    for (int b = 0; b < NB; ++b) {
        Blk& k = blk_[b];
        k.ln1 = carve(nullptr, BT * d); k.ln1_mean = carve(nullptr, BT); k.ln1_rstd = carve(nullptr, BT);
        k.q = carve(nullptr, BT * 3 * d); k.k = k.q + d; k.v = k.q + 2 * d;
        k.lse = carve(nullptr, B * NH * (size_t)T); k.ao = carve(nullptr, BT * d); k.x1 = carve(nullptr, BT * d);
        k.ln2 = carve(nullptr, BT * d); k.ln2_mean = carve(nullptr, BT); k.ln2_rstd = carve(nullptr, BT);
        k.cq = carve(nullptr, BT * d); k.ck = carve(nullptr, BK * d); k.cv = carve(nullptr, BK * d);
        k.cP = carve(nullptr, B * NH * (size_t)T * K); k.cao = carve(nullptr, BT * d); k.x2 = carve(nullptr, BT * d);
        k.ln3 = carve(nullptr, BT * d); k.ln3_mean = carve(nullptr, BT); k.ln3_rstd = carve(nullptr, BT);
        k.f1 = carve(fmt("blk%d.ffn_hidden", b).c_str(), BT * 4 * d); k.x3 = carve(nullptr, BT * d);
    }
    bg_.resize(NB);
    {
        const size_t NC = xattn_supported(K, d, NH) ? (size_t)NH * xattn_kp(K, NH) : 16;
        xa_zero_base_ = carve_pos();
        for (int b = 0; b < NB; ++b) {
            Blk& k = blk_[b];
            k.xaAb = carve(nullptr, B * NC * d); k.xaAbT = carve(nullptr, B * NC * d); k.xaVo = carve(nullptr, B * NC * d); k.xaVoT = carve(nullptr, B * NC * d);
        }
        xa_zero_floats_ = (size_t)(carve_pos() - xa_zero_base_);
        for (int b = 0; b < NB; ++b) { bg_[b].xaPd = carve(nullptr, BT * NC); bg_[b].xaDs = carve(nullptr, BT * NC); }
        xa_dAb_ = carve(nullptr, B * NC * d); xa_dVo_ = carve(nullptr, B * NC * d);
        xa_pq_ = carve(nullptr, B * (size_t)d * d); xa_po_ = carve(nullptr, B * (size_t)d * d);
    }
    attn_delta_ = carve(nullptr, B * NH * (size_t)T);
    attn_ds_ = attn_ds_floats_ ? carve(nullptr, attn_ds_floats_) : nullptr;
    lnf_ =carve("dec_out", BT * d); lnf_mean_ = carve(nullptr, BT); lnf_rstd_ = carve(nullptr, BT);
    pred_ = carve("pred", BT * V);
    gx_ = carve(nullptr, BT * d); gbr_ = carve(nullptr, BT * d); gt1_ = carve(nullptr, BT * d); gt2_ = carve(nullptr, BT * d);
    gt3_ = carve(nullptr, BT * d); gf1_ = carve(nullptr, BT * 4 * d); gqkv_ = carve(nullptr, BT * 3 * d);
    for (int b = 0; b < NB; ++b) {
        BlkG& q = bg_[b];
        if (b == 0) { q.gbr[0] = gbr_; q.gf1 = gf1_; q.gt2 = gt2_; q.gqkv = gqkv_; }
        else { q.gbr[0] = carve(nullptr, BT * d); q.gf1 = carve(nullptr, BT * 4 * d); q.gt2 = carve(nullptr, BT * d); q.gqkv = carve(nullptr, BT * 3 * d); }
        q.gbr[1] = carve(nullptr, BT * d); q.gbr[2] = carve(nullptr, BT * d);
    }
    scratch3_ = carve(nullptr, scratch_floats_);
    gmem_ = carve(nullptr, BK * d); gck_ = carve(nullptr, BK * d); gcv_ = carve(nullptr, BK * d);
    gdA_ = carve(nullptr, BN * 64); gdB_ = carve(nullptr, BN * 64);
    }
    col0_ = dw0p_ = nullptr;
    if (!first_direct()) {
        const int ldc0 = (25 * cfg.obs_channels + 3) & ~3;
        col0_ = carve(nullptr, BN * ldc0); dw0p_ = carve(nullptr, (size_t)64 * ldc0);
    }
    end_layout();
}

int SlateModel::bind(float* p, float* g, float* m, float* v, void* ws, size_t ws_bytes) {
    RC(check_buffers(p, g, ws, ws_bytes));
    OCRL_REQUIRE(d % 64 == 0 && d <= 256 && D % 64 == 0 && C == 64 && V % 256 == 0 && S % 4 == 0 && d % NH == 0 && DH % 4 == 0 && DH <= 64,
                 "unsupported configuration (d_model/slot_size multiples of 64 <= 256, cnn hidden 64, vocab %% 256, obs_size %% 4)");
    OCRL_REQUIRE(cfg.obs_channels == 3, "obs_channels must be 3");
    OCRL_REQUIRE(T % 4 == 0, "obs_size/4 squared must be a multiple of 4");
    adopt_buffers(p, g, m, v, ws);
    clear_encode_graphs();
    packs_valid_ = false;
    layout_workspace(true);
    if (!side_) {
        plan_ = stream_plan((int)sw::model<sw::OCRL_OVERLAP>(), (int)sw::model<sw::OCRL_DW_SIDE>(), sw::model<sw::OCRL_TOKENS_LATE>() != 0, cfg.use_bcdec);
        if (plan_.side) {
            OCRL_HIP(hipStreamCreateWithFlags(&side_, hipStreamNonBlocking));
            OCRL_HIP(hipEventCreateWithFlags(&ev_fork_, hipEventDisableTiming));
            OCRL_HIP(hipEventCreateWithFlags(&ev_join_, hipEventDisableTiming));
            OCRL_HIP(hipEventCreateWithFlags(&ev_tokens_, hipEventDisableTiming));
            if (plan_.dw) {
                for (hipEvent_t& ev : ev_dw_) OCRL_HIP(hipEventCreateWithFlags(&ev, hipEventDisableTiming));
                OCRL_HIP(hipEventCreateWithFlags(&ev_join2_, hipEventDisableTiming));
                if (plan_.dw == 2) OCRL_HIP(hipStreamCreateWithFlags(&side2_, hipStreamNonBlocking));
            }
        }
    }
    sa_input_ = (int)sw::model<sw::OCRL_SA_INPUT>();
    xattn_ = !cfg.use_bcdec && xattn_supported(K, d, NH) && sw::model<sw::OCRL_XATTN>() != 0;
    if (!cfg.use_bcdec && xa_zero_floats_) OCRL_HIP(hipMemset(xa_zero_base_, 0, xa_zero_floats_ * sizeof(float)));
    RC(posgrid_launch(gridT_, S, 0));
    RC(fill_launch(recon_, (long long)Bmax * N * 4, 0.f, 0));
    const float* saw[SA_NW];
    for (int i = 0; i < SA_NW; ++i) saw[i] = P(w_.sa.w[i]);
    PackEntry ent[SA_PACK_ENTRIES];
    sa_pack_n_ = sa_pack_table(saw, C, D, H, ent, &sa_pack_max_);
    OCRL_HIP(hipMemcpy(sa_pack_dev_, ent, sa_pack_n_ * sizeof(PackEntry), hipMemcpyHostToDevice));
    OCRL_HIP(hipDeviceSynchronize());
    have_fwd_ = false;
    return 0;
}

int SlateModel::soft_z(hipStream_t st) {
    if (!fused_heads() || cfg.use_bcdec) return 0;
    OCRL_REQUIRE(have_scores_, "soft_z: no forward since the last backward (the scores have been overwritten by their gradient)");
    return exp_rows_launch(zraw_, zlse_, z_, (long long)last_.B * T, V, st);
}
int SlateModel::dropout_mask(unsigned site, long long n, float* out, hipStream_t st) const {
    return dropout_mask_launch(out, n, pdrop_, last_.seed, site, st);
}

int SlateModel::conv_layer_fwd(const float* x, const float* pack, const float* bias, float* y, int Bn, int Hh, int Ww, int KS, int CIN,
                               int relu, const float* posmap, const float* mask, const Lane& L) {
    ConvArgs a;
    a.X = x; a.Wp = pack; a.Y = y; a.B = Bn; a.H = Hh; a.W = Ww; a.bias = bias; a.relu = relu; a.posmap = posmap; a.mask = mask;
    if (conv_x3_ > 0 && (KS == 5 || KS == 3) && CIN == 64 && !conv_lowlat_) {
        auto it = x3_of_.find(pack);
        if (it != x3_of_.end()) return conv_x3_launch(a, it->second, L, KS);
    }
    return conv_fwd_launch(a, KS, CIN, 64, L, conv_lowlat_);
}
int SlateModel::conv_layer_wgrad(const float* x, const float* dy, float* dW, float* db, int Bn, int Hh, int Ww, int KS, int CIN,
                                 int cin_real, const Lane& L) {
    WgradArgs a;
    a.X = x; a.dY = dy; a.part = L.scratch; a.B = Bn; a.H = Hh; a.W = Ww;
    OCRL_REQUIRE(conv_wgrad_ws_floats(Bn, Hh, Ww, KS, CIN) <= L.scratch_floats, "conv wgrad: scratch too small");
    const bool x3 = conv_x3_ > 0 && CIN == 64;
    RC(conv_wgrad_launch(a, KS, CIN, 64, cin_real, dW, x3 ? nullptr : db, 0, L, x3 ? 1 : 0));
    if (db && x3) RC(colsum_launch(dy, 64, db, (long long)Bn * Hh * Ww, 64, 0, 1.f, L.scratch, L.scratch_floats, L));
    return 0;
}

int SlateModel::pack_weights(const Lane& L, bool encoder_only) {
    if (first_direct()) RC(conv_first_pack_launch(P(w_.enc[0].w), cw_fwd_[0], L));
    else RC(conv_pack_launch(P(w_.enc[0].w), cw_fwd_[0], nullptr, 5, 8, 64, cfg.obs_channels, L));
    RC(conv_pack_launch(P(w_.enc[1].w), cw_fwd_[1], cw_bwd_[1], 5, 64, 64, 64, L));
    RC(conv_pack_launch(P(w_.enc[2].w), cw_fwd_[2], cw_bwd_[2], 5, 64, 64, 64, L));
    RC(conv_pack_launch(P(w_.enc[3].w), cw_fwd_[3], cw_bwd_[3], 5, 64, 64, 64, L));
    if (conv_x3_ > 0) {
        for (int i = 1; i < 4; ++i) {
            auto f = x3_of_.find(cw_fwd_[i]), b = x3_of_.find(cw_bwd_[i]);
            if (f != x3_of_.end()) RC(conv_pack_x3_launch(P(w_.enc[i].w), const_cast<float*>(f->second), b != x3_of_.end() ? const_cast<float*>(b->second) : nullptr, L));
        }
    }
    if (!cfg.use_bcdec && !encoder_only) {
        RC(conv_pack_launch(P(w_.dvae_dec[1].w), dw_fwd_[0], dw_bwd_[0], 3, 64, 64, 64, L));
        RC(conv_pack_launch(P(w_.dvae_dec[6].w), dw_fwd_[1], dw_bwd_[1], 3, 64, 64, 64, L));
        if (conv_x3_ > 0) {
            for (int i = 0; i < 2; ++i) {
                auto f = x3_of_.find(dw_fwd_[i]), b = x3_of_.find(dw_bwd_[i]);
                if (f != x3_of_.end()) RC(conv_pack_x3_launch(P(w_.dvae_dec[i ? 6 : 1].w), const_cast<float*>(f->second), b != x3_of_.end() ? const_cast<float*>(b->second) : nullptr, L, 3));
            }
        }
        RC(copy_launch(P(w_.dvae_dec[11].w), w11p_, cfg.obs_channels * 64, L));
        RC(fill_launch(w11p_ + cfg.obs_channels * 64, (4 - cfg.obs_channels) * 64, 0.f, L));
    }
    RC(pack_launch(sa_pack_dev_, sa_pack_n_, sa_pack_max_, sa_wts_, L));
    RC(posmap_launch(P(w_.enc_pos.w), P(w_.enc_pos.b), posmap_, S, C, L));
    return 0;
}

int SlateModel::fwd_encoder(const StepInputs& in, const Lane& L, FwdDvae fork) {
    const int B = in.B;
    const long long BN = (long long)B * N;
    auto fork_if = [&](FwdDvae here) -> int {
        if (fork != here) return 0;
        RC(after(dvae_lane(), L, ev_fork_));
        return fwd_dvae(in, dvae_lane());
    };
    RC(slot_init_launch(P(w_.sa.mu), P(w_.sa.log_sigma), in.noise_slots, slots0_, B * K, D, in.seed, L, in.seed_dev));
    SlotAttnArgs a = sa_args(B, N, K, D, H, I, SH);
    a.x = x_; a.slots0 = slots0_; a.wts = sa_wts_; a.slots = slots_; a.attn = attn_; a.attn_heads = attn_heads_; a.save = sa_save_;
    if (conv_lowlat_ && frozen_) a.save = nullptr;
    a.xchg = sa_xchg_; a.parts = sa_parts_;
    a.phase = 1;
    RC(slot_attn_launch(a, 0, L));
    RC(fork_if(FwdDvae::AtStart));
    if (first_direct()) {
        RC(conv_first_fwd_launch(in.obs, cw_fwd_[0], P(w_.enc[0].b), e1_, B, S, S, 1, L));
        if (!(conv_lowlat_ && frozen_))
            OCRL_HIP(hipMemcpyAsync(obs_keep_, in.obs, (size_t)BN * cfg.obs_channels * sizeof(float), hipMemcpyDeviceToDevice, L));
    } else {
        RC(nchw_to_nhwc8_launch(in.obs, obs8_, B, cfg.obs_channels, S, S, L));
        RC(conv_layer_fwd(obs8_, cw_fwd_[0], P(w_.enc[0].b), e1_, B, S, S, 5, 8, 1, nullptr, nullptr, L));
    }
    RC(conv_layer_fwd(e1_, cw_fwd_[1], P(w_.enc[1].b), e2_, B, S, S, 5, 64, 1, nullptr, nullptr, L));
    RC(conv_layer_fwd(e2_, cw_fwd_[2], P(w_.enc[2].b), e3_, B, S, S, 5, 64, 1, nullptr, nullptr, L));
    RC(conv_layer_fwd(e3_, cw_fwd_[3], P(w_.enc[3].b), e4_, B, S, S, 5, 64, 0, posmap_, nullptr, L));
    RC(fork_if(FwdDvae::AfterConvs));
    if (sa_input_ && C == 64 && !(conv_lowlat_ && frozen_)) {
        RC(sa_input_fwd_launch(e4_, P(w_.sa.ln.w), P(w_.sa.ln.b), P(w_.sa.mlp0.w),
                               P(w_.sa.mlp0.b), P(w_.sa.mlp2.w), P(w_.sa.mlp2.b), ln0_mean_, ln0_rstd_,
                               sa_input_ == 2 ? ln0_ : nullptr, h1_, x_, BN, 0, L));
    } else {
        RC(layernorm_fwd_launch(e4_, P(w_.sa.ln.w), P(w_.sa.ln.b), ln0_, ln0_mean_, ln0_rstd_, BN, C, L));
        RC(lin_fwd(ln0_, C, P(w_.sa.mlp0.w), P(w_.sa.mlp0.b), h1_, C, BN, C, C, 1, nullptr, 0, 0.f, 0, L));
        RC(lin_fwd(h1_, C, P(w_.sa.mlp2.w), P(w_.sa.mlp2.b), x_, C, BN, C, C, 0, nullptr, 0, 0.f, 0, L));
    }
    RC(fork_if(FwdDvae::AtSlotAttention));
    a.phase = 2;
    RC(slot_attn_launch(a, 0, L));
    return 0;
}

int SlateModel::fwd_dvae(const StepInputs& in, const Lane& L) {
// ... 132 lines not shown
    OCRL_REQUIRE(p_ && ws_, "forward: model not bound");
    OCRL_REQUIRE(in.B >= 1 && in.B <= Bmax, "forward: batch %d outside [1,%d]", in.B, Bmax);
    OCRL_REQUIRE(in.obs && in.tau > 0.f, "forward: bad inputs");
    last_ = in;
    have_enc_ = false;
    pdrop_ = in.train ? cfg.dropout : 0.f;
    const Lane L = main_lane(st);
    RC(pack_weights(L));
    if (cfg.use_bcdec) {
        RC(fwd_encoder(in, L));
        RC(pack_bcdec(L));
        RC(fwd_bcdec(L));
        RC(fill_launch(metrics_ + 1, 1, 0.f, L));
        RC(copy_launch(metrics_ + 0, metrics_ + 2, 1, L));
        have_fwd_ = true;
        return 0;
    }
    if (plan_.fwd_dvae == FwdDvae::Serial) RC(fwd_dvae(in, L));
    if (plan_.fwd_dvae == FwdDvae::BesideEncoder) {
        RC(after(dvae_lane(), L, ev_fork_));
        RC(fwd_dvae(in, dvae_lane()));
    }
    RC(fwd_encoder(in, L, plan_.fwd_dvae));
    if (plan_.tokens_early) OCRL_HIP(hipStreamWaitEvent(L, ev_tokens_, 0));
    else if (plan_.side) RC(after(L, dvae_lane(), ev_join_));
    RC(fwd_decoder(L));
    if (plan_.tokens_early) RC(after(L, dvae_lane(), ev_join_));
    RC(copy_launch(metrics_ + 0, metrics_ + 2, 1, L));
    RC(axpy_launch(metrics_ + 1, metrics_ + 2, 1, 1.f, L));
    have_fwd_ = true;
    return 0;
}

int SlateModel::encode(const StepInputs& in, hipStream_t st) {
    OCRL_REQUIRE(p_ && ws_, "encode: model not bound");
    OCRL_REQUIRE(in.B >= 1 && in.B <= Bmax && in.obs, "encode: bad inputs");
    last_ = in;
    pdrop_ = 0.f;
    have_fwd_ = false;
    have_enc_ = true;
    const Lane L = main_lane(st);
    if (enc_graph_mode_ < 0) enc_graph_mode_ = (int)sw::model<sw::OCRL_ENCODE_GRAPH>();
    const bool graph = enc_graph_mode_ && in.B <= 32 && !in.noise_slots && obs_stage_;
    const bool need_pack = !(frozen_ && packs_valid_);
    struct LowLat { int& f; LowLat(int& x) : f(x) { f = 1; } ~LowLat() { f = 0; } } lowlat(conv_lowlat_);
    if (!graph) {
        if (need_pack) RC(pack_weights(L, true));
        packs_valid_ = frozen_;
        return fwd_encoder(in, L);
    }
    EncGraph& eg = enc_graphs_[in.B];
    if (!eg.warm || need_pack) {
        eg.warm = 1;
        if (need_pack) RC(pack_weights(L, true));
        packs_valid_ = frozen_;
        return fwd_encoder(in, L);
    }
    const size_t bytes = (size_t)in.B * cfg.obs_channels * N * sizeof(float);
    OCRL_HIP(hipMemcpyAsync(obs_stage_, in.obs, bytes, hipMemcpyDeviceToDevice, L));
    RC(store_u64_launch(seed_dev_, in.seed, L));
    if (!eg.exec) {
        StepInputs gi = in;
        gi.obs = obs_stage_; gi.seed_dev = seed_dev_;
        hipGraph_t g = nullptr;
        if (!cap_) OCRL_HIP(hipStreamCreateWithFlags(&cap_, hipStreamNonBlocking));
        OCRL_HIP(hipStreamBeginCapture(cap_, hipStreamCaptureModeThreadLocal));
        const Lane cap = main_lane(cap_);
        int rc = frozen_ ? 0 : pack_weights(cap, true);
        if (!rc) rc = fwd_encoder(gi, cap);
        const hipError_t ce = hipStreamEndCapture(cap_, &g);
        if (rc) { if (g) (void)hipGraphDestroy(g); return rc; }
        OCRL_HIP(ce);
        OCRL_HIP(hipGraphInstantiate(&eg.exec, g, nullptr, nullptr, 0));
        OCRL_HIP(hipGraphDestroy(g));
    }
    OCRL_HIP(hipGraphLaunch(eg.exec, L));
    return 0;
}

void SlateModel::clear_encode_graphs() {
    for (auto& kv : enc_graphs_) if (kv.second.exec) (void)hipGraphExecDestroy(kv.second.exec);
    enc_graphs_.clear();
}

int SlateModel::encode_backward(const float* dslots, hipStream_t st) {
    OCRL_REQUIRE(have_enc_, "encode_backward: call encode first (its activations are what is differentiated)");
    OCRL_REQUIRE(!frozen_, "encode_backward: the weights are frozen (ocrl_slate_freeze_weights): encode() kept no activations");
    OCRL_REQUIRE(g_ && dslots, "encode_backward: no gradient buffer bound / null dslots");
    const Lane L = main_lane(st);
    RC(fill_launch(g_, flat_size_, 0.f, L));
    RC(copy_launch(dslots, gslots_, (long long)last_.B * K * D, L));
    RC(bwd_encoder(L));
    have_enc_ = false;
    enc_only_grads_ = true;
    return 0;
}

int SlateModel::generate(hipStream_t st) {
    OCRL_REQUIRE(!cfg.use_bcdec, "generate: the autoregressive decoder is not part of the use_bcdec configuration");
    OCRL_REQUIRE(last_.B > 0 && last_.obs, "generate: run forward or encode first");
    have_enc_ = false;
    const int B = last_.B;
    const long long BK = (long long)B * K;
    pdrop_ = 0.f;
    have_fwd_ = false;
    const Lane L = main_lane(st);
    OCRL_HIP(hipMemsetAsync(tokens_, 0, sizeof(int) * (size_t)B * T, L));
    RC(lin_fwd(slots_, D, P(w_.slotproj), nullptr, mem_, d, BK, d, D, 0, nullptr, 0, 0.f, 0, L));
    for (int b = 0; b < NB; ++b) {
        const DecBlockW& bw = w_.blk[b];
        RC(lin_fwd(mem_, d, P(bw.ck), nullptr, blk_[b].ck, d, BK, d, d, 0, nullptr, 0, 0.f, 0, L));
        RC(lin_fwd(mem_, d, P(bw.cv), nullptr, blk_[b].cv, d, BK, d, d, 0, nullptr, 0, 0.f, 0, L));
    }
    float* x0 = emb_;
    for (int t = 0; t < T; ++t) {
        RC(embed_step_launch(tokens_, P(w_.dict), P(w_.bos), P(w_.pe), x0, B, T, d, t, L));
        const float* xin = x0;
        for (int b = 0; b < NB; ++b) {
            Blk& k = blk_[b];
            const DecBlockW& bw = w_.blk[b];
            RC(layernorm_fwd_launch(xin, P(bw.ln1.w), P(bw.ln1.b), k.ln1, k.ln1_mean, k.ln1_rstd, B, d, L));
            const float* res = (b == 0) ? k.ln1 : xin;
            RC(lin_fwd(k.ln1, d, P(bw.qkv), nullptr, k.q + (size_t)t * 3 * d, T * 3 * d, B, 3 * d, d, 0, nullptr, 0, 0.f, 0, L));
            RC(decode_attn_launch(k.q, k.ao, B, T, t, d, NH, 3 * d, L));
            RC(lin_fwd(k.ao, d, P(bw.o), nullptr, k.x1, d, B, d, d, 0, res, d, 0.f, 0, L));
            RC(layernorm_fwd_launch(k.x1, P(bw.ln2.w), P(bw.ln2.b), k.ln2, k.ln2_mean, k.ln2_rstd, B, d, L));
            RC(lin_fwd(k.ln2, d, P(bw.cq), nullptr, k.cq, d, B, d, d, 0, nullptr, 0, 0.f, 0, L));
            RC(cross_attn_fwd_launch(k.cq, k.ck, k.cv, k.cao, k.cP, B, 1, K, d, NH, 0.f, 0, 0, L));
            RC(lin_fwd(k.cao, d, P(bw.co), nullptr, k.x2, d, B, d, d, 0, k.x1, d, 0.f, 0, L));
            RC(layernorm_fwd_launch(k.x2, P(bw.ln3.w), P(bw.ln3.b), k.ln3, k.ln3_mean, k.ln3_rstd, B, d, L));
            RC(lin_fwd(k.ln3, d, P(bw.ffn0.w), P(bw.ffn0.b), k.f1, 4 * d, B, 4 * d, d, 1, nullptr, 0, 0.f, 0, L));
            RC(lin_fwd(k.f1, 4 * d, P(bw.ffn2.w), P(bw.ffn2.b), k.x3, d, B, d, 4 * d, 0, k.x2, d, 0.f, 0, L));
            xin = k.x3;
        }
        RC(layernorm_fwd_launch(xin, P(w_.lnf.w), P(w_.lnf.b), lnf_, lnf_mean_, lnf_rstd_, B, d, L));
        RC(lin_fwd(lnf_, d, P(w_.out), nullptr, pred_, V, B, V, d, 0, nullptr, 0, 0.f, 0, L));
        RC(argmax_pos_launch(pred_, tokens_, B, T, V, t, L, 1));
    }
    RC(onehot_launch(tokens_, z_, (long long)B * T, V, L));
    RC(dvae_decode(B, nullptr, L, z_));
    return 0;
}

int SlateModel::bwd_decoder(const Lane& L) {
    const int B = last_.B;
    const long long BT = (long long)B * T, BK = (long long)B * K;
    const float p = pdrop_;
    const Lane W = dw_lane(L);
    const bool dws = plan_.dw != 0;
    Xf ce; ce.a_mode = 3; ce.lse = celse_; ce.tok = tokens_; ce.scale = 1.0f / last_.B;
    RC(after(W, L, ring_event()));
    RC(lin_bwd_w(pred_, V, lnf_, d, G(w_.out), nullptr, BT, V, d, 1.f, W, ce));
    RC(lin_bwd_x(pred_, V, P(w_.out), gt1_, d, BT, V, d, nullptr, 0, nullptr, 0, L, Drop(), ce));
    const float* xlast = blk_[NB - 1].x3;
    RC(layernorm_bwd_launch(gt1_, xlast, lnf_mean_, lnf_rstd_, P(w_.lnf.w), gx_, G(w_.lnf.w), BT, d, 0, 0,
                            L.scratch, L.scratch_floats, L));
    RC(fill_launch(gmem_, BK * d, 0.f, L));
    for (int b = NB - 1; b >= 0; --b) {
        Blk& k = blk_[b];
        const BlkG& q = bg_[dws ? b : 0];
        const DecBlockW& bw = w_.blk[b];
        const unsigned site = SITE_BLK_BASE + 8 * b;
        const float* xin = (b == 0) ? emb_ : blk_[b - 1].x3;
        const float* gd = gx_;
        auto drop_gx = [&](unsigned s_, float* into) -> int {
            gd = gx_;
            if (p > 0.f || dws) { RC(dropout_apply_launch(gx_, into, BT * d, p, last_.seed, s_, L)); gd = into; }
            return 0;
        };
        RC(drop_gx(site + 4, q.gbr[0]));
        RC(lin_bwd_x(gd, d, P(bw.ffn2.w), q.gf1, 4 * d, BT, d, 4 * d, k.f1, 4 * d, nullptr, 0, L));
        RC(after(W, L, ring_event()));
        RC(lin_bwd_w(gd, d, k.f1, 4 * d, G(bw.ffn2.w), G(bw.ffn2.b), BT, d, 4 * d, 1.f, W));
        RC(lin_bwd_w(q.gf1, 4 * d, k.ln3, d, G(bw.ffn0.w), G(bw.ffn0.b), BT, 4 * d, d, 1.f, W));
        RC(lin_bwd_x(q.gf1, 4 * d, P(bw.ffn0.w), gt1_, d, BT, 4 * d, d, nullptr, 0, nullptr, 0, L));
        RC(layernorm_bwd_launch(gt1_, k.x2, k.ln3_mean, k.ln3_rstd, P(bw.ln3.w), gx_, G(bw.ln3.w), BT, d, 1, 0,
                                L.scratch, L.scratch_floats, L));
        RC(drop_gx(site + 3, q.gbr[1]));
        const float* gd_co = gd;
        if (xattn_) {
            XaHost hx = xattn_args(b);
            hx.y = gt1_; hx.gd = gd_co; hx.Pd = q.xaPd; hx.dS = q.xaDs;
            RC(xattn_launch(hx, 1, L));
            RC(after(W, L, ring_event()));
            XaFoldBwdHost f;
            f.Pd = q.xaPd; f.dS = q.xaDs; f.gd = gd_co; f.x = k.ln2; f.Wq = P(bw.cq); f.Wo = P(bw.co); f.ck = k.ck; f.cv = k.cv;
            f.dVo = xa_dVo_; f.dAb = xa_dAb_; f.dck = gck_; f.dcv = gcv_; f.pq = xa_pq_; f.po = xa_po_; f.dWq = G(bw.cq); f.dWo = G(bw.co);
            f.ws = W.scratch; f.ws_floats = W.scratch_floats; f.B = B; f.T = T; f.K = K; f.d = d; f.h = NH;
            RC(xattn_fold_bwd_launch(f, W));
        } else {
        RC(lin_bwd_x(gd, d, P(bw.co), gt1_, d, BT, d, d, nullptr, 0, nullptr, 0, L));
        RC(cross_attn_bwd_launch(gt1_, k.cq, k.ck, k.cv, k.cP, q.gt2, gck_, gcv_, B, T, K, d, NH, p, last_.seed, site + 2, L.scratch, L.scratch_floats, L));
        RC(after(W, L, ring_event()));
        RC(lin_bwd_w(gd_co, d, k.cao, d, G(bw.co), nullptr, BT, d, d, 1.f, W));
        RC(lin_bwd_w(q.gt2, d, k.ln2, d, G(bw.cq), nullptr, BT, d, d, 1.f, W));
        RC(lin_bwd_x(q.gt2, d, P(bw.cq), gt1_, d, BT, d, d, nullptr, 0, nullptr, 0, L));
        }
        {
            const Lane& X = xattn_ ? W : L;
            RC(lin_bwd_w(gck_, d, mem_, d, G(bw.ck), nullptr, BK, d, d, 1.f, X));
            RC(lin_bwd_w(gcv_, d, mem_, d, G(bw.cv), nullptr, BK, d, d, 1.f, X));
            RC(lin_bwd_x(gck_, d, P(bw.ck), gmem_, d, BK, d, d, nullptr, 0, gmem_, d, X));
            RC(lin_bwd_x(gcv_, d, P(bw.cv), gmem_, d, BK, d, d, nullptr, 0, gmem_, d, X));
        }
        RC(layernorm_bwd_launch(gt1_, k.x1, k.ln2_mean, k.ln2_rstd, P(bw.ln2.w), gx_,
                                G(bw.ln2.w), BT, d, 1, 0, L.scratch, L.scratch_floats, L));
        RC(drop_gx(site + 1, q.gbr[2]));
        const float* gd_o = gd;
        RC(lin_bwd_x(gd, d, P(bw.o), gt1_, d, BT, d, d, nullptr, 0, nullptr, 0, L));
        {
            AttnArgs a = self_attn_args(b);
            a.dO = gt1_; a.dq = q.gqkv; a.dk = q.gqkv + d; a.dv = q.gqkv + 2 * d; a.delta = attn_delta_;
            a.ds = attn_ds_; a.ds_floats = attn_ds_floats_;
            RC(attn_launch(a, 1, L));
        }
        RC(after(W, L, ring_event()));
        RC(lin_bwd_w(gd_o, d, k.ao, d, G(bw.o), nullptr, BT, d, d, 1.f, W));
        RC(lin_bwd_w(q.gqkv, 3 * d, k.ln1, d, G(bw.qkv), nullptr, BT, 3 * d, d, 1.f, W));
        RC(lin_bwd_x(q.gqkv, 3 * d, P(bw.qkv), gt1_, d, BT, 3 * d, d, nullptr, 0, nullptr, 0, L));
        if (b == 0) {
            RC(axpy_launch(gx_, gt1_, BT * d, 1.f, L));
            RC(layernorm_bwd_launch(gt1_, xin, k.ln1_mean, k.ln1_rstd, P(bw.ln1.w), gx_,
                                    G(bw.ln1.w), BT, d, 0, 0, L.scratch, L.scratch_floats, L));
        } else {
            RC(layernorm_bwd_launch(gt1_, xin, k.ln1_mean, k.ln1_rstd, P(bw.ln1.w), gx_,
                                    G(bw.ln1.w), BT, d, 1, 0, L.scratch, L.scratch_floats, L));
        }
    }
    RC(embed_bwd_launch(gx_, tokens_, G(w_.dict), B, T, V, d, p, last_.seed, L.scratch, L.scratch_floats, L));
    RC(fill_launch(G(w_.pe), (long long)(T + 1) * d, 0.f, L));
    RC(colsum_launch(gx_, (long long)T * d, G(w_.pe), B, T * d, 0, 1.f, L.scratch, L.scratch_floats, L));
    RC(copy_launch(G(w_.pe), G(w_.bos), d, L));
    if (xattn_) RC(after(L, W, ring_event()));
    RC(lin_bwd_w(gmem_, d, slots_, D, G(w_.slotproj), nullptr, BK, d, D, 1.f, L));
    RC(lin_bwd_x(gmem_, d, P(w_.slotproj), gslots_, D, BK, d, D, nullptr, 0, nullptr, 0, L));
    return 0;
}

int SlateModel::bwd_encoder(const Lane& L, BwdDvae fork) {
    const bool fork_dvae = fork == BwdDvae::AtSlotAttention;
    const int B = last_.B;
    const long long BN = (long long)B * N, R = (long long)B * I * K;
    const SlotAttnW& sa = w_.sa;
    SlotAttnArgs a = sa_args(B, N, K, D, H, I, SH);
    a.x = x_; a.wts = sa_wts_; a.save = sa_save_; a.dslots = gslots_; a.dx = gA_; a.dslots0 = gslots0_; a.grows = sa_grows_; a.g_small = sa_small_;
    a.xchg = sa_xchg_; a.parts = sa_parts_;
    if (fork_dvae) {
        RC(after(dvae_lane(), L, ev_fork_));
        RC(bwd_dvae(dvae_lane()));
    }
    RC(slot_attn_launch(a, 1, L));
    const bool side_w = plan_.sa_wgrads_on_side;
    const Lane W = side_w ? dvae_lane() : L;
    if (side_w) RC(after(W, L, ev_fork_));
    const bool sa_in_bwd = sa_input_ == 1 && C == 64;
    SaWgrad wg[SA_MAX_WGRADS];
    const int nwg = sa_wgrad_list(C, D, H, SH, a.scale, wg);
    for (int i = 0; i < nwg; ++i) {
        const SaWgrad& e = wg[i];
        RC(lin_bwd_w(e.dy.at(sa_save_, sa_grows_), e.dy.ld, e.x.at(sa_save_, sa_grows_), e.x.ld, G(sa.w[e.w]) + e.w_off,
                     e.b < 0 ? nullptr : G(sa.w[e.b]), R, e.N_out, e.K_in, e.alpha, W));
    }
    const int SM = 4 * D + 2 * C;
    RC(colsum_launch(sa_small_ + 0, SM, G(sa.w[SAW_NORM_SLOTS_W]), B, 2 * D, 0, 1.f, W.scratch, W.scratch_floats, W));
    RC(colsum_launch(sa_small_ + 2 * D, SM, G(sa.w[SAW_NORM_MLP_W]), B, 2 * D, 0, 1.f, W.scratch, W.scratch_floats, W));
    RC(colsum_launch(sa_small_ + 4 * D, SM, G(sa.w[SAW_NORM_INPUTS_W]), B, 2 * C, 0, 1.f, W.scratch, W.scratch_floats, W));
    RC(slot_init_bwd_launch(gslots0_, P(w_.sa.log_sigma), last_.noise_slots, G(w_.sa.mu), G(w_.sa.log_sigma),
                            B * K, D, last_.seed, W));
    if (!sa_in_bwd) RC(lin_bwd_w(gA_, C, h1_, C, G(w_.sa.mlp2.w), G(w_.sa.mlp2.b), BN, C, C, 1.f, W));
    if (side_w && !first_direct()) RC(im2col5_launch(obs8_, col0_, BN, S, S, cfg.obs_channels, (25 * cfg.obs_channels + 3) & ~3, W));
    if (sa_in_bwd) {
        const size_t slabs = L.scratch_floats / SA_INPUT_SLAB;
        OCRL_REQUIRE(slabs >= 1, "bwd_encoder: scratch too small for the input-chain slabs");
        RC(sa_input_bwd_launch(gA_, h1_, e4_, ln0_mean_, ln0_rstd_, P(w_.sa.ln.w), P(w_.sa.ln.b),
                               P(w_.sa.mlp0.w), P(w_.sa.mlp2.w), gB_, G(w_.sa.mlp0.w), G(w_.sa.mlp0.b),
                               G(w_.sa.mlp2.w), G(w_.sa.mlp2.b), G(w_.sa.ln.w), G(w_.sa.ln.b),
                               BN, slabs < 512 ? (int)slabs : 0, L.scratch, L.scratch_floats, L));
    } else {
        RC(lin_bwd_x(gA_, C, P(w_.sa.mlp2.w), gB_, C, BN, C, C, h1_, C, nullptr, 0, L));
        RC(lin_bwd_w(gB_, C, ln0_, C, G(w_.sa.mlp0.w), G(w_.sa.mlp0.b), BN, C, C, 1.f, L));
        float* gL = side_w ? gC_ : gA_;
        RC(lin_bwd_x(gB_, C, P(w_.sa.mlp0.w), gL, C, BN, C, C, nullptr, 0, nullptr, 0, L));
        RC(layernorm_bwd_launch(gL, e4_, ln0_mean_, ln0_rstd_, P(w_.sa.ln.w), gB_, G(w_.sa.ln.w), BN, C, 0, 0,
                                L.scratch, L.scratch_floats, L));
    }
    RC(colsum_launch(gB_, (long long)N * C, gmap_, B, N * C, 0, 1.f, L.scratch, L.scratch_floats, L));
    RC(lin_bwd_w(gmap_, C, gridT_, 4, G(w_.enc_pos.w), G(w_.enc_pos.b), N, C, 4, 1.f, L));
    if (fork_dvae || side_w) RC(after(L, dvae_lane(), ev_join_));
    if (plan_.dw == 2) RC(after(L, dw_lane(L), ev_join2_));
    RC(colsum_launch(gmap_, C, G(w_.enc[3].b), N, C, 0, 1.f, L.scratch, L.scratch_floats, L));
    RC(conv_layer_wgrad(e3_, gB_, G(w_.enc[3].w), nullptr, B, S, S, 5, 64, 64, L));
    RC(conv_layer_fwd(gB_, cw_bwd_[3], nullptr, gA_, B, S, S, 5, 64, 0, nullptr, e3_, L));
    RC(conv_layer_wgrad(e2_, gA_, G(w_.enc[2].w), G(w_.enc[2].b), B, S, S, 5, 64, 64, L));
    RC(conv_layer_fwd(gA_, cw_bwd_[2], nullptr, gB_, B, S, S, 5, 64, 0, nullptr, e2_, L));
    RC(conv_layer_wgrad(e1_, gB_, G(w_.enc[1].w), G(w_.enc[1].b), B, S, S, 5, 64, 64, L));
    RC(conv_layer_fwd(gB_, cw_bwd_[1], nullptr, gA_, B, S, S, 5, 64, 0, nullptr, e1_, L));
    if (first_direct()) {
        OCRL_REQUIRE(conv_first_wgrad_ws_floats(B, S, S) <= L.scratch_floats, "first conv wgrad: scratch too small");
        RC(conv_first_wgrad_launch(obs_keep_, gA_, L.scratch, G(w_.enc[0].w), G(w_.enc[0].b), B, S, S, 0, L));
    } else {
        const int ch = cfg.obs_channels, ldc0 = (25 * ch + 3) & ~3;
        if (!side_w) RC(im2col5_launch(obs8_, col0_, BN, S, S, ch, ldc0, L));
        RC(lin_bwd_w(gA_, 64, col0_, ldc0, dw0p_, G(w_.enc[0].b), BN, 64, ldc0, 1.f, L));
        RC(unpack5_launch(dw0p_, G(w_.enc[0].w), ch, ldc0, L));
    }
    return 0;
}

int SlateModel::bwd_dvae(const Lane& L) {
    const int B = last_.B;
    const long long BT = (long long)B * T, BN = (long long)B * N;
    const int ch = cfg.obs_channels;
    float* w4 = L.scratch + L.scratch_floats - 1024;
    {
        GemmArgs a;
        a.A = drecon_; a.B = ps2_; a.C = w4; a.M = 4; a.N = 64; a.K = (int)BN; a.lda = 4; a.ldb = 64; a.ldc = 64; a.akc = 0; a.bkc = 0;
        long long splits = BN / 512; if (splits > 512) splits = 512; if (splits < 1) splits = 1;
        if (splits > 1) {
            a.splitk = (int)splits; a.C = L.scratch; a.sCsplit = 256;
            RC(gemm_launch(a, L));
            RC(splitk_reduce_launch(L.scratch, w4, 256, (int)splits, 256, 0, L));
        } else RC(gemm_launch(a, L));
        RC(copy_launch(w4, G(w_.dvae_dec[11].w), ch * 64, L));
        RC(colsum_launch(drecon_, 4, w4 + 256, BN, 4, 0, 1.f, L.scratch, L.scratch_floats - 1024, L));
        RC(copy_launch(w4 + 256, G(w_.dvae_dec[11].b), ch, L));
    }
    RC(lin_bwd_x(drecon_, 4, w11p_, gdA_, 64, BN, 4, 64, nullptr, 0, nullptr, 0, L));
    RC(pixel_shuffle_launch(gdA_, gdB_, B, 2 * E, 2 * E, 64, 0, dd9_, L));
    RC(lin_bwd_w(gdB_, 256, dd8_, 64, G(w_.dvae_dec[9].w), G(w_.dvae_dec[9].b), 4 * BT, 256, 64, 1.f, L));
    RC(lin_bwd_x(gdB_, 256, P(w_.dvae_dec[9].w), gdA_, 64, 4 * BT, 256, 64, dd8_, 64, nullptr, 0, L));
    RC(lin_bwd_w(gdA_, 64, dd7_, 64, G(w_.dvae_dec[8].w), G(w_.dvae_dec[8].b), 4 * BT, 64, 64, 1.f, L));
    RC(lin_bwd_x(gdA_, 64, P(w_.dvae_dec[8].w), gdB_, 64, 4 * BT, 64, 64, dd7_, 64, nullptr, 0, L));
    RC(lin_bwd_w(gdB_, 64, dd6_, 64, G(w_.dvae_dec[7].w), G(w_.dvae_dec[7].b), 4 * BT, 64, 64, 1.f, L));
    RC(lin_bwd_x(gdB_, 64, P(w_.dvae_dec[7].w), gdA_, 64, 4 * BT, 64, 64, dd6_, 64, nullptr, 0, L));
    RC(conv_layer_wgrad(ps1_, gdA_, G(w_.dvae_dec[6].w), G(w_.dvae_dec[6].b), B, 2 * E, 2 * E, 3, 64, 64, L));
    RC(conv_layer_fwd(gdA_, dw_bwd_[1], nullptr, gdB_, B, 2 * E, 2 * E, 3, 64, 0, nullptr, ps1_, L));
    RC(pixel_shuffle_launch(gdB_, gdA_, B, E, E, 64, 0, nullptr, L));
    RC(lin_bwd_w(gdA_, 256, dd3_, 64, G(w_.dvae_dec[4].w), G(w_.dvae_dec[4].b), BT, 256, 64, 1.f, L));
    RC(lin_bwd_x(gdA_, 256, P(w_.dvae_dec[4].w), gdB_, 64, BT, 256, 64, dd3_, 64, nullptr, 0, L));
    RC(lin_bwd_w(gdB_, 64, dd2_, 64, G(w_.dvae_dec[3].w), G(w_.dvae_dec[3].b), BT, 64, 64, 1.f, L));
    RC(lin_bwd_x(gdB_, 64, P(w_.dvae_dec[3].w), gdA_, 64, BT, 64, 64, dd2_, 64, nullptr, 0, L));
    RC(lin_bwd_w(gdA_, 64, dd1_, 64, G(w_.dvae_dec[2].w), G(w_.dvae_dec[2].b), BT, 64, 64, 1.f, L));
    RC(lin_bwd_x(gdA_, 64, P(w_.dvae_dec[2].w), gdB_, 64, BT, 64, 64, dd1_, 64, nullptr, 0, L));
    RC(conv_layer_wgrad(dd0_, gdB_, G(w_.dvae_dec[1].w), G(w_.dvae_dec[1].b), B, E, E, 3, 64, 64, L));
    RC(conv_layer_fwd(gdB_, dw_bwd_[0], nullptr, gdA_, B, E, E, 3, 64, 0, nullptr, dd0_, L));
    float* dz = zraw_;
    have_scores_ = false;
    if (fused_heads()) {
        Xf zx; zx.b_mode = 2; zx.lse = zlse_;
        RC(lin_bwd_w(gdA_, 64, zraw_, V, G(w_.dvae_dec[0].w), G(w_.dvae_dec[0].b), BT, 64, V, 1.f, L, zx));
        RC(rowdot_bias64_launch(gdA_, dd0_, P(w_.dvae_dec[0].b), BT, zdot_, L));
        GemmArgs a;
        a.A = gdA_; a.B = P(w_.dvae_dec[0].w); a.C = dz; a.M = (int)BT; a.N = V; a.K = 64; a.lda = 64; a.ldb = V; a.ldc = V; a.bkc = 0;
        a.epi_mode = 3; a.mask = zraw_; a.ldmask = V; a.e_lse = zlse_; a.e_rowvec = zdot_; a.e_scale = 1.0f / last_.tau;
        RC(gemm_launch(a, L));
    } else {
    RC(lin_bwd_w(gdA_, 64, zdec_, V, G(w_.dvae_dec[0].w), G(w_.dvae_dec[0].b), BT, 64, V, 1.f, L));
    RC(lin_bwd_x(gdA_, 64, P(w_.dvae_dec[0].w), dz, V, BT, 64, V, nullptr, 0, nullptr, 0, L));
    RC(softmax_bwd_rows_launch(z_, dz, BT, V, 1.0f / last_.tau, L));
    }
    RC(lin_bwd_w(dz, V, de_[6], 64, G(w_.dvae_enc[7].w), G(w_.dvae_enc[7].b), BT, V, 64, 1.f, L));
    RC(lin_bwd_x(dz, V, P(w_.dvae_enc[7].w), gdA_, 64, BT, V, 64, de_[6], 64, nullptr, 0, L));
    float* cur = gdA_;
    float* oth = gdB_;
    for (int i = 6; i >= 1; --i) {
        RC(lin_bwd_w(cur, 64, de_[i - 1], 64, G(w_.dvae_enc[i].w), G(w_.dvae_enc[i].b), BT, 64, 64, 1.f, L));
        RC(lin_bwd_x(cur, 64, P(w_.dvae_enc[i].w), oth, 64, BT, 64, 64, de_[i - 1], 64, nullptr, 0, L));
        float* t = cur; cur = oth; oth = t;
    }
    RC(lin_bwd_w(cur, 64, patches_, 16 * ch, G(w_.dvae_enc[0].w), G(w_.dvae_enc[0].b), BT, 64, 16 * ch, 1.f, L));
    return 0;
}

int SlateModel::backward(hipStream_t st) {
    OCRL_REQUIRE(have_fwd_, "backward: call forward first");
    OCRL_REQUIRE(g_, "backward: no gradient buffer bound");
    enc_only_grads_ = false;
    const Lane L = main_lane(st);
    if (cfg.use_bcdec) {
        RC(fill_launch(g_, flat_size_, 0.f, L));
        RC(bwd_bcdec(L));
        RC(bwd_encoder(L));
        have_fwd_ = false;
        return 0;
    }
    const BwdDvae at = plan_.bwd_dvae;
    if (at == BwdDvae::BesideAll || at == BwdDvae::BesideDecoder) {
        RC(after(dvae_lane(), L, ev_fork_));
// ... 91 lines not shown
```

ocrl_amd/csrc/slate_model.h:

```cpp
#pragma once
#include <map>
#include <string>
#include <vector>

#include "kernels.h"
#include "model_base.h"
#include "slot_attn_host.h"
#include "stream_plan.h"

struct SlateConfig {
    int obs_size = 64, obs_channels = 3, vocab = 4096, d_model = 192, cnn_hidden = 64;
    int num_slots = 5, num_iters = 3, slot_size = 192, mlp_hidden = 192;
    int num_blocks = 4, num_heads = 4;
    float dropout = 0.1f;
    int max_batch = 1;
    int use_bcdec = 0;
    int hard = 0;
    int slot_heads = 1;
};

struct StepInputs {
    const float* obs = nullptr;
    int B = 0;
    float tau = 1.f;
// ... 4 lines not shown
    const float* noise_slots = nullptr;
    const unsigned long long* seed_dev = nullptr;
};

struct Lane {
    hipStream_t st = nullptr;
    float* scratch = nullptr;
    size_t scratch_floats = 0;
    operator hipStream_t() const { return st; }
};

class SlateModel : public ModelBase {
public:
    explicit SlateModel(const SlateConfig& c);
    ~SlateModel();
    long long group_begin(int g) const { return group_begin_[g]; }
    int bind(float* p, float* g, float* m, float* v, void* ws, size_t ws_bytes);
    int forward(const StepInputs& in, hipStream_t st);
    int backward(hipStream_t st);
    int encode(const StepInputs& in, hipStream_t st);
    void freeze_weights(bool on) { frozen_ = on; packs_valid_ = false; clear_encode_graphs(); }
    void clear_encode_graphs();
    int encode_backward(const float* dslots, hipStream_t st);
    int generate(hipStream_t st);
    int clip_adam(const float lr[3], float clip, int step, float gscale, hipStream_t st);
    int grad_norm(hipStream_t st);
    int dropout_mask(unsigned site, long long n, float* out, hipStream_t st) const;
    int soft_z(hipStream_t st);
    const SlateConfig cfg;

private:
    void layout_workspace(bool commit);
    int lin_fwd(const float* x, int ldx, const float* W, const float* b, float* y, int ldy, long long M, int N, int K, int relu,
                const float* resid, int ldr, float drop_p, unsigned site, hipStream_t st) {
        return ::lin_fwd(x, ldx, W, b, y, ldy, M, N, K, relu, resid, ldr, st, Drop{drop_p, last_.seed, site});
    }
    int lin_bwd_w(const float* dy, int ld_dy, const float* x, int ldx, float* dW, float* db, long long M, int N_out, int K_in,
                  float alpha, const Lane& L, Xf xf = Xf()) {
        return ::lin_bwd_w(dy, ld_dy, x, ldx, dW, db, M, N_out, K_in, alpha, L.scratch, L.scratch_floats, L.st, Drop(), xf);
    }
    bool fused_heads() const { return !cfg.hard; }
    int conv_layer_fwd(const float* x, const float* pack, const float* bias, float* y, int Bn, int Hh, int Ww, int KS, int CIN, int relu,
                       const float* posmap, const float* mask, const Lane& L);
    int conv_layer_wgrad(const float* x, const float* dy, float* dW, float* db, int Bn, int Hh, int Ww, int KS, int CIN, int cin_real,
                         const Lane& L);
    int pack_weights(const Lane& L, bool encoder_only = false);
    int fwd_encoder(const StepInputs& in, const Lane& L, FwdDvae fork = FwdDvae::Serial);
    int fwd_dvae(const StepInputs& in, const Lane& L);
    int fwd_decoder(const Lane& L, bool with_ce = true);
    int dvae_decode(int B, float* drecon, const Lane& L, const float* zin = nullptr);
    int bwd_decoder(const Lane& L);
    int bwd_encoder(const Lane& L, BwdDvae fork = BwdDvae::SerialLast);
    int bwd_dvae(const Lane& L);
    int pack_bcdec(const Lane& L);
    int fwd_bcdec(const Lane& L);
    int bwd_bcdec(const Lane& L);
    AttnArgs self_attn_args(int b) const;
    XaHost xattn_args(int b) const;

    Lane main_lane(hipStream_t st) const { return Lane{st, scratch_, scratch_floats_}; }
    Lane dvae_lane() const { return Lane{side_, scratch2_, scratch_floats_}; }
    Lane dw_lane(const Lane& main) const { return plan_.dw == 2 ? Lane{side2_, scratch3_, scratch_floats_} : plan_.dw ? dvae_lane() : main; }
    int after(const Lane& waiter, const Lane& producer, hipEvent_t ev);
    hipEvent_t ring_event() { return ev_dw_[ev_dw_next_++ & 7]; }

    struct DecBlockW { ParamPair ln1, ln2, ln3, ffn0, ffn2; ParamRef qkv, o, cq, ck, cv, co; };
    struct SlotAttnW {
        ParamRef mu, log_sigma;
        ParamPair ln, mlp0, mlp2;
        ParamRef w[SA_NW];
    };
    struct Weights {
        ParamPair dvae_enc[8], dvae_dec[12];
        ParamPair enc[4], enc_pos;
        SlotAttnW sa;
        ParamPair bc[4], bc_pos;
        ParamRef slotproj, dict, bos, pe, out;
        ParamPair lnf;
        std::vector<DecBlockW> blk;
        long long enc_grads_end = 0;
    } w_;
    void resolve_params();

    long long group_begin_[4] = {0, 0, 0, 0};

    int S, E, T, N, V, d, C, K, I, D, H, NB, NH, DH, Bmax;
    int SH = 1;
    StepInputs last_;
    float pdrop_ = 0.f;
    bool have_fwd_ = false;
    int conv_lowlat_ = 0;
    bool frozen_ = false, packs_valid_ = false;
    bool have_enc_ = false;
    bool enc_only_grads_ = false;
    bool have_scores_ = false;

    float *scratch_ = nullptr;
    size_t scratch_floats_ = 0;
    float* scratch2_ = nullptr;
    StreamPlan plan_;
    hipStream_t side_ = nullptr;
    hipEvent_t ev_fork_ = nullptr, ev_join_ = nullptr, ev_tokens_ = nullptr;
    float *zstat_ = nullptr, *zhstat_ = nullptr, *zlse_ = nullptr, *zdot_ = nullptr, *cestat_ = nullptr, *celse_ = nullptr, *cepart_ = nullptr;
    int* zhidx_ = nullptr;
    float *obs8_, *patches_, *de_[7], *zraw_, *z_, *zdec_;
    int* tokens_;
    float *dd0_, *dd1_, *dd2_, *dd3_, *dd4_, *ps1_, *dd6_, *dd7_, *dd8_, *dd9_, *ps2_, *recon_, *drecon_;
    float *e1_, *e2_, *e3_, *e4_, *posmap_, *gridT_, *ln0_, *ln0_mean_, *ln0_rstd_, *h1_, *x_;
    float *slots0_, *slot_noise_, *slots_, *attn_, *sa_save_, *sa_wts_, *sa_grows_, *sa_small_, *sa_xchg_;
    float* attn_heads_ = nullptr;
    float* sa_parts_;
    PackEntry* sa_pack_dev_ = nullptr;
    int sa_pack_n_ = 0, sa_pack_max_ = 0;
    float *cw_fwd_[4], *cw_bwd_[4];
    int conv_x3_ = 0;
    std::map<const float*, const float*> x3_of_;
    float *dw_fwd_[2], *dw_bwd_[2];
    float *w11p_;
    float *mem_, *emb_;
    struct Blk {
        float *ln1, *ln1_mean, *ln1_rstd, *q, *k, *v, *lse, *ao, *x1;
        float *ln2, *ln2_mean, *ln2_rstd, *cq, *ck, *cv, *cP, *cao, *x2;
        float *ln3, *ln3_mean, *ln3_rstd, *f1, *x3;
        float *xaAb, *xaAbT, *xaVo, *xaVoT;
    };
    int sa_input_ = 1;
    bool xattn_ = false;
    float *xa_dAb_ = nullptr, *xa_dVo_ = nullptr, *xa_pq_ = nullptr, *xa_po_ = nullptr;
    size_t xa_zero_floats_ = 0;
    float* xa_zero_base_ = nullptr;
    std::vector<Blk> blk_;
    struct BlkG { float *gbr[3], *gf1, *gt2, *gqkv, *xaPd, *xaDs; };
    std::vector<BlkG> bg_;
    struct EncGraph { hipGraphExec_t exec = nullptr; int warm = 0; };
    std::map<int, EncGraph> enc_graphs_;
    int enc_graph_mode_ = -1;
    hipStream_t cap_ = nullptr;
    float* obs_stage_ = nullptr;
    unsigned long long* seed_dev_ = nullptr;
    hipStream_t side2_ = nullptr;
    float* scratch3_ = nullptr;
    hipEvent_t ev_dw_[8] = {nullptr, nullptr, nullptr, nullptr, nullptr, nullptr, nullptr, nullptr};
    hipEvent_t ev_join2_ = nullptr;
    int ev_dw_next_ = 0;
    float *attn_delta_;
    float *attn_ds_ = nullptr;
    size_t attn_ds_floats_ = 0;
    float *lnf_, *lnf_mean_, *lnf_rstd_, *pred_;
    float *gqkv_;
    float *gx_, *gbr_, *gt1_, *gt2_, *gt3_, *gf1_, *gmem_, *gck_, *gcv_, *gslots_, *gslots0_;
    float *gA_, *gB_, *gC_;
    float *gdA_, *gdB_;
    float *gmap_;
    float *col0_, *dw0p_;
    float* obs_keep_ = nullptr;
    bool first_direct() const { return cfg.obs_channels == 3; }
    float *bc_Wc_, *bc_W1r_, *bc_P1_, *bc_M_, *bc_T_, *bc_c1_, *bc_c2_, *bc_c3_, *bc_out4_, *bc_dout4_, *bc_gA_, *bc_gB_;
    float *bc_pk_[2], *bc_pkb_[2], *bc_Wk4_, *bc_Wb4_, *bc_dW1r_, *bc_dWc_, *bc_dT_, *bc_dM_, *bc_G1_;
};
```

Baseline: 1793.

## Fuse dropout and residual add into LayerNorm backward, batch gamma/beta colsums

```diff
diff --git a/include/ocrl_hip_ln_tails.h b/include/ocrl_hip_ln_tails.h
--- /dev/null
+++ b/include/ocrl_hip_ln_tails.h
@@ -0,0 +1,30 @@
+#ifndef OCRL_HIP_LN_TAILS_H
+#define OCRL_HIP_LN_TAILS_H
+#include <stddef.h>
+
+#ifdef __cplusplus
+extern "C" {
+#endif
+
+typedef struct {
+    const float* X;
+    long long ld;
+    float* out;
+    long long R;
+    int F;
+    int accumulate;
+    float* ws;
+    size_t ws_floats;
+} ocrl_lt_site;
+
+int ocrl_lt_site_size(void);
+int ocrl_lt_layernorm_bwd_blocks(long long R, int F, size_t part_floats);
+int ocrl_lt_layernorm_bwd(const float* dy, const float* dy2 , const float* x, const float* mean, const float* rstd,
+                          const float* gamma, float* dx, float* drop , long long R, int F, int accumulate_dx, float p,
+                          unsigned long long seed, unsigned site, float* part, size_t part_floats, int nblk[1], void* stream);
+int ocrl_lt_colsum_table(const ocrl_lt_site* sites, int n, void* stream);
+
+#ifdef __cplusplus
+}
+#endif
+#endif
diff --git a/ocrl_amd/_lib.py b/ocrl_amd/_lib.py
--- a/ocrl_amd/_lib.py
+++ b/ocrl_amd/_lib.py
@@ -16,6 +16,7 @@
 IODINE_HEADER_PATH = os.path.join(_HERE, os.pardir, "include", "ocrl_hip_iodine.h")
 QR_HEADER_PATH = os.path.join(_HERE, os.pardir, "include", "ocrl_hip_qr.h")
 SLATE_KERNELS_HEADER_PATH = os.path.join(_HERE, os.pardir, "include", "ocrl_hip_slate_kernels.h")
+LN_TAILS_HEADER_PATH = os.path.join(_HERE, os.pardir, "include", "ocrl_hip_ln_tails.h")
 _lib = None
 
 if not os.path.exists(HEADER_PATH):
@@ -69,6 +70,11 @@
     raise RuntimeError(f"{SLATE_KERNELS_HEADER_PATH} is missing: ocrl_amd derives its binding of libocrl_hip.so from the header and runs from the source tree.")
 with open(SLATE_KERNELS_HEADER_PATH) as _f:
     ABI_SLATE_KERNELS = _abi.read(_f.read())
+if not os.path.exists(LN_TAILS_HEADER_PATH):
+    raise RuntimeError(f"{LN_TAILS_HEADER_PATH} is missing: ocrl_amd derives its binding of libocrl_hip.so from the header and runs from the source tree.")
+with open(LN_TAILS_HEADER_PATH) as _f:
+    ABI_LN_TAILS = _abi.read(_f.read())
+LnSite = ABI_LN_TAILS.structs["ocrl_lt_site"]
 
 
 def flat_segments(segs):
@@ -155,14 +161,14 @@
             "(make -C ocrl_amd/csrc).  ocrl_amd has no CPU fallback.")
     import torch
     L = ctypes.CDLL(LIB_PATH)
-    for abi in (ABI, ABI_DQN, ABI_ROLLOUT, ABI_REPLAY, ABI_C51, ABI_NOISY, ABI_CLASSIFIER, ABI_IODINE, ABI_QR, ABI_SLATE_KERNELS):
+    for abi in (ABI, ABI_DQN, ABI_ROLLOUT, ABI_REPLAY, ABI_C51, ABI_NOISY, ABI_CLASSIFIER, ABI_IODINE, ABI_QR, ABI_SLATE_KERNELS, ABI_LN_TAILS):
         for name, (restype, argtypes) in abi.functions.items():
             f = getattr(L, name)
             f.argtypes = argtypes
             if restype is not ctypes.c_int:
                 f.restype = restype
-    for name, cls in {**ABI.structs, **ABI_DQN.structs, **ABI_C51.structs, **ABI_NOISY.structs, **ABI_QR.structs}.items():
-        if name + "_size" in {**ABI.functions, **ABI_DQN.functions, **ABI_C51.functions, **ABI_NOISY.functions, **ABI_QR.functions} and getattr(L, name + "_size")() != ctypes.sizeof(cls):
+    for name, cls in {**ABI.structs, **ABI_DQN.structs, **ABI_C51.structs, **ABI_NOISY.structs, **ABI_QR.structs, **ABI_LN_TAILS.structs}.items():
+        if name + "_size" in {**ABI.functions, **ABI_DQN.functions, **ABI_C51.functions, **ABI_NOISY.functions, **ABI_QR.functions, **ABI_LN_TAILS.functions} and getattr(L, name + "_size")() != ctypes.sizeof(cls):
             raise RuntimeError(f"libocrl_hip.so: {name} is {getattr(L, name + '_size')()} bytes, this binding's {cls.__name__} {ctypes.sizeof(cls)}")
     if L.ocrl_abi_version() != CONSTANTS["OCRL_ABI_VERSION"]:
         raise RuntimeError(f"libocrl_hip.so ABI version mismatch: the library is {L.ocrl_abi_version()}, include/ocrl_hip.h {CONSTANTS['OCRL_ABI_VERSION']}")
diff --git a/ocrl_amd/csrc/elementwise.hip b/ocrl_amd/csrc/elementwise.hip
--- a/ocrl_amd/csrc/elementwise.hip
+++ b/ocrl_amd/csrc/elementwise.hip
@@ -106,10 +106,40 @@
     }
 }
 
-template <int NPL>
+struct LnBwdTail {
+    const float* dy2;
+    float* drop;
+    float p;
+    unsigned long long seed;
+    unsigned site;
+};
+template <int W, bool TAIL>
+__device__ __forceinline__ void layernorm_bwd_store(float (&o)[W], float* dx, long long e, int accumulate, const LnBwdTail& t) {
+    static_assert(W == 1 || W == 4, "one float or one float4");
+    if (accumulate) {
+        if constexpr (W == 4) { const float4 a = *reinterpret_cast<const float4*>(dx + e); o[0] += a.x; o[1] += a.y; o[2] += a.z; o[3] += a.w; }
+        else o[0] = dx[e] + o[0];
+    }
+    if constexpr (W == 4) *reinterpret_cast<float4*>(dx + e) = make_float4(o[0], o[1], o[2], o[3]);
+    else dx[e] = o[0];
+    if constexpr (TAIL) {
+        if (!t.drop) return;
+        if (t.p > 0.f) {
+            const uint2 bits = rng_bits4(t.seed, t.site, (uint64_t)(e >> 2));
+            const uint32_t thr = drop_thresh(t.p);
+            const float sc = 1.0f / (1.0f - t.p);
+#pragma unroll
+            for (int j = 0; j < W; ++j) o[j] = rng_keep(bits, (int)((e + j) & 3), thr) ? o[j] * sc : 0.f;
+        }
+        if constexpr (W == 4) *reinterpret_cast<float4*>(t.drop + e) = make_float4(o[0], o[1], o[2], o[3]);
+        else t.drop[e] = o[0];
+    }
+}
+
+template <int NPL, bool TAIL>
 __global__ void layernorm_bwd_kernel(const float* __restrict__ dy, const float* __restrict__ x, const float* __restrict__ mean,
-                                     const float* __restrict__ rstd, const float* __restrict__ g, float* __restrict__ dx,
-                                     float* __restrict__ part, long long R, int accumulate) {
+                                     const float* __restrict__ rstd, const float* __restrict__ g, float* dx,
+                                     float* __restrict__ part, long long R, int accumulate, LnBwdTail tail) {
     constexpr int F = 64 * NPL;
     __shared__ float red[4][2 * F];
     const int lane = threadIdx.x & 63, wv = threadIdx.x >> 6;
@@ -120,24 +150,53 @@
         const float mu = mean[row], rs = rstd[row];
         float xh[NPL], d[NPL];
         float s1 = 0.f, s2 = 0.f;
-#pragma unroll
-        for (int i = 0; i < NPL; ++i) {
-            const int c = i * 64 + lane;
-            xh[i] = (x[row * F + c] - mu) * rs;
-            const float dyv = dy[row * F + c];
-            dg[i] += dyv * xh[i];
-            db[i] += dyv;
-            d[i] = dyv * gg[i];
-            s1 += d[i];
-            s2 += d[i] * xh[i];
-        }
-        s1 = wave_sum(s1) * (1.0f / F);
-        s2 = wave_sum(s2) * (1.0f / F);
-#pragma unroll
-        for (int i = 0; i < NPL; ++i) {
-            const int c = i * 64 + lane;
-            const float v = rs * (d[i] - s1 - xh[i] * s2);
-            dx[row * F + c] = accumulate ? dx[row * F + c] + v : v;
+        if constexpr (TAIL) {
+#pragma clang fp contract(off)
+            constexpr float inv_f = 1.0f / F;
+            float dyv[NPL];
+#pragma unroll
+            for (int i = 0; i < NPL; ++i) {
+                const int c = i * 64 + lane;
+                xh[i] = (x[row * F + c] - mu) * rs;
+                dyv[i] = dy[row * F + c];
+                if (tail.dy2) dyv[i] += tail.dy2[row * F + c];
+                if constexpr (NPL == 1) dg[i] += dyv[i] * xh[i];
+                else dg[i] = fmaf(dyv[i], xh[i], dg[i]);
+                db[i] += dyv[i];
+                d[i] = dyv[i] * gg[i];
+                if (NPL == 4 && i == 1) { s1 = fmaf(dyv[i], gg[i], s1); s2 = fmaf(d[i], xh[i], s2); }
+                else { s1 += d[i]; s2 += d[i] * xh[i]; }
+            }
+            const float S1 = wave_sum(s1), S2 = wave_sum(s2);
+            const float s1m = S1 * inv_f, s2m = S2 * inv_f;
+#pragma unroll
+            for (int i = 0; i < NPL; ++i) {
+                const long long e = row * F + i * 64 + lane;
+                const float t = i == 0 ? fmaf(S1, -inv_f, d[i]) : d[i] - s1m;
+                const float u = fmaf(-s2m, xh[i], t);
+                float v[1] = {rs * u};
+                layernorm_bwd_store<1, TAIL>(v, dx, e, accumulate, tail);
+            }
+        } else {
+#pragma unroll
+            for (int i = 0; i < NPL; ++i) {
+                const int c = i * 64 + lane;
+                xh[i] = (x[row * F + c] - mu) * rs;
+                const float dyv = dy[row * F + c];
+                dg[i] += dyv * xh[i];
+                db[i] += dyv;
+                d[i] = dyv * gg[i];
+                s1 += d[i];
+                s2 += d[i] * xh[i];
+            }
+            s1 = wave_sum(s1) * (1.0f / F);
+            s2 = wave_sum(s2) * (1.0f / F);
+#pragma unroll
+            for (int i = 0; i < NPL; ++i) {
+                const int c = i * 64 + lane;
+                float v[1] = {rs * (d[i] - s1 - xh[i] * s2)};
+                layernorm_bwd_store<1, TAIL>(v, dx, row * F + c, accumulate, tail);
+            }
         }
     }
 #pragma unroll
@@ -179,10 +238,10 @@
         }
     }
 }
-template <int NV, int NP>
+template <int NV, int NP, bool TAIL>
 __global__ __launch_bounds__(256) void layernorm16_bwd_kernel(const float* __restrict__ dy, const float* __restrict__ x, const float* __restrict__ mean,
-                                                              const float* __restrict__ rstd, const float* __restrict__ g, float* __restrict__ dx,
-                                                              float* __restrict__ part, long long R, int accumulate) {
+                                                              const float* __restrict__ rstd, const float* __restrict__ g, float* dx,
+                                                              float* __restrict__ part, long long R, int accumulate, LnBwdTail tail) {
     constexpr int F = 64 * NV;
     __shared__ float4 red[2][16][16 * NV];
     const int lane = threadIdx.x & 63, wv = threadIdx.x >> 6, c4 = lane & 15, rsub = lane >> 4;
@@ -201,6 +260,12 @@
             for (int k = 0; k < NV; ++k) {
                 xv[i][k] = ok ? *reinterpret_cast<const float4*>(x + row * F + (k * 16 + c4) * 4) : make_float4(0.f, 0.f, 0.f, 0.f);
                 yv[i][k] = ok ? *reinterpret_cast<const float4*>(dy + row * F + (k * 16 + c4) * 4) : make_float4(0.f, 0.f, 0.f, 0.f);
+                if constexpr (TAIL) {
+                    if (tail.dy2 && ok) {
+                        const float4 b = *reinterpret_cast<const float4*>(tail.dy2 + row * F + (k * 16 + c4) * 4);
+                        yv[i][k].x += b.x; yv[i][k].y += b.y; yv[i][k].z += b.z; yv[i][k].w += b.w;
+                    }
+                }
             }
             mu[i] = ok ? mean[row] : 0.f;
             rs[i] = ok ? rstd[row] : 0.f;
@@ -212,10 +277,9 @@
             if (row < R) {
 #pragma unroll
                 for (int k = 0; k < NV; ++k) {
-                    float4 o = layernorm16_row_dx(r, rs[i], k);
-                    float* dp = dx + row * F + (k * 16 + c4) * 4;
-                    if (accumulate) { const float4 a = *reinterpret_cast<const float4*>(dp); o.x += a.x; o.y += a.y; o.z += a.z; o.w += a.w; }
-                    *reinterpret_cast<float4*>(dp) = o;
+                    const float4 o4 = layernorm16_row_dx(r, rs[i], k);
+                    float o[4] = {o4.x, o4.y, o4.z, o4.w};
+                    layernorm_bwd_store<4, TAIL>(o, dx, row * F + (k * 16 + c4) * 4, accumulate, tail);
                 }
             }
         }
@@ -232,24 +296,27 @@
     }
 }
 
-__global__ void colsum_kernel(const float* __restrict__ X, long long ld, float* __restrict__ part, long long R, int F, long long rows_per_chunk) {
-    __shared__ float red[4][64];
+__device__ __forceinline__ void colsum_body(const float* __restrict__ X, long long ld, float* __restrict__ part, long long R, int F, long long rows_per_chunk,
+                                            int chunk, float (*red)[64]) {
     const int col = blockIdx.x * 64 + (threadIdx.x & 63), rl = threadIdx.x >> 6;
-    const long long r0 = (long long)blockIdx.y * rows_per_chunk;
+    const long long r0 = (long long)chunk * rows_per_chunk;
     const long long r1 = min(R, r0 + rows_per_chunk);
     float s = 0.f;
     if (col < F)
         for (long long r = r0 + rl; r < r1; r += 4) s += X[r * ld + col];
     red[rl][threadIdx.x & 63] = s;
     __syncthreads();
-    if (rl == 0 && col < F) part[(size_t)blockIdx.y * F + col] = red[0][threadIdx.x] + red[1][threadIdx.x] + red[2][threadIdx.x] + red[3][threadIdx.x];
-}
-__global__ __launch_bounds__(256) void colsum4_kernel(const float* __restrict__ X, long long ld, float* __restrict__ part, long long R, int F,
-                                                      long long rows_per_chunk) {
-    __shared__ float4 red[256];
+    if (rl == 0 && col < F) part[(size_t)chunk * F + col] = red[0][threadIdx.x] + red[1][threadIdx.x] + red[2][threadIdx.x] + red[3][threadIdx.x];
+}
+__global__ void colsum_kernel(const float* __restrict__ X, long long ld, float* __restrict__ part, long long R, int F, long long rows_per_chunk) {
+    __shared__ float red[4][64];
+    colsum_body(X, ld, part, R, F, rows_per_chunk, blockIdx.y, red);
+}
+__device__ __forceinline__ void colsum4_body(const float* __restrict__ X, long long ld, float* __restrict__ part, long long R, int F, long long rows_per_chunk,
+                                             int chunk, float4* red) {
     const int F4 = F >> 2, RL = 256 / F4;
     const int c4 = threadIdx.x % F4, rl = threadIdx.x / F4;
-    const long long r0 = (long long)blockIdx.x * rows_per_chunk;
+    const long long r0 = (long long)chunk * rows_per_chunk;
     const long long r1 = min(R, r0 + rows_per_chunk);
     float4 s0 = make_float4(0.f, 0.f, 0.f, 0.f), s1 = s0, s2 = s0, s3 = s0;
     if (rl < RL) {
@@ -273,11 +340,16 @@
     if (threadIdx.x < F4) {
         float4 t = red[threadIdx.x];
         for (int k = 1; k < RL; ++k) { const float4 v = red[k * F4 + threadIdx.x]; t.x += v.x; t.y += v.y; t.z += v.z; t.w += v.w; }
-        *reinterpret_cast<float4*>(part + (size_t)blockIdx.x * F + threadIdx.x * 4) = t;
-    }
-}
-__global__ __launch_bounds__(256) void colsum_final_kernel(const float* __restrict__ part, float* __restrict__ out, int nchunk, int F, int accumulate, float scale) {
-    __shared__ float red[16][16];
+        *reinterpret_cast<float4*>(part + (size_t)chunk * F + threadIdx.x * 4) = t;
+    }
+}
+__global__ __launch_bounds__(256) void colsum4_kernel(const float* __restrict__ X, long long ld, float* __restrict__ part, long long R, int F,
+                                                      long long rows_per_chunk) {
+    __shared__ float4 red[256];
+    colsum4_body(X, ld, part, R, F, rows_per_chunk, blockIdx.x, red);
+}
+__device__ __forceinline__ void colsum_final_body(const float* __restrict__ part, float* __restrict__ out, int nchunk, int F, int accumulate, float scale,
+                                                  float (*red)[16]) {
     const int cl = threadIdx.x & 15, rl = threadIdx.x >> 4;
     const int c = blockIdx.x * 16 + cl;
     float s0 = 0.f, s1 = 0.f;
@@ -295,6 +367,34 @@
         t *= scale;
         out[c] = accumulate ? out[c] + t : t;
     }
+}
+__global__ __launch_bounds__(256) void colsum_final_kernel(const float* __restrict__ part, float* __restrict__ out, int nchunk, int F, int accumulate, float scale) {
+    __shared__ float red[16][16];
+    colsum_final_body(part, out, nchunk, F, accumulate, scale, red);
+}
+struct ColsumSite {
+    const float* X; long long ld; float* part; float* out; long long R; long long rpc;
+    int F, nchunk, accumulate, vec4;
+};
+constexpr int COLSUM_TABLE_MAX = 16;
+struct ColsumTable { ColsumSite s[COLSUM_TABLE_MAX]; };
+__global__ __launch_bounds__(256) void colsum4_table_kernel(ColsumTable t) {
+    __shared__ float4 red[256];
+    const ColsumSite& s = t.s[blockIdx.y];
+    if (!s.vec4 || (int)blockIdx.x >= s.nchunk) return;
+    colsum4_body(s.X, s.ld, s.part, s.R, s.F, s.rpc, blockIdx.x, red);
+}
+__global__ __launch_bounds__(256) void colsum_table_kernel(ColsumTable t) {
+    __shared__ float red[4][64];
+    const ColsumSite& s = t.s[blockIdx.z];
+    if (s.vec4 || (int)blockIdx.y >= s.nchunk || (int)blockIdx.x * 64 >= s.F) return;
+    colsum_body(s.X, s.ld, s.part, s.R, s.F, s.rpc, blockIdx.y, red);
+}
+__global__ __launch_bounds__(256) void colsum_final_table_kernel(ColsumTable t) {
+    __shared__ float red[16][16];
+    const ColsumSite& s = t.s[blockIdx.y];
+    if ((int)blockIdx.x * 16 >= s.F) return;
+    colsum_final_body(s.part, s.out, s.nchunk, s.F, s.accumulate, 1.f, red);
 }
 
 __global__ void reduce_partials_kernel(const float* __restrict__ part, int n, float* __restrict__ out, float scale, int accumulate) {
@@ -952,19 +1052,15 @@
     OCRL_CHECK_LAUNCH("layernorm_fwd");
     return 0;
 }
-int colsum_launch(const float* X, long long ld, float* out, long long R, int F, int accumulate, float scale, float* ws, size_t ws_floats, hipStream_t st) {
+struct ColsumPlan { bool vec4; long long nchunk, rpc; };
+static ColsumPlan colsum_plan(const float* X, long long ld, long long R, int F, size_t ws_floats) {
     if (F % 4 == 0 && ld % 4 == 0 && F <= 1024 && F >= 4 && (((uintptr_t)X) & 15) == 0 && R >= 1024) {
         long long nchunk = 2048;
         if (nchunk > R / 8) nchunk = R / 8;
         if ((size_t)nchunk * F > ws_floats) nchunk = (long long)(ws_floats / F);
         if (nchunk >= 16) {
             const long long rpc = (R + nchunk - 1) / nchunk;
-            nchunk = (R + rpc - 1) / rpc;
-            hipLaunchKernelGGL(colsum4_kernel, dim3((unsigned)nchunk), dim3(256), 0, st, X, ld, ws, R, F, rpc);
-            OCRL_CHECK_LAUNCH("colsum4");
-            hipLaunchKernelGGL(colsum_final_kernel, dim3(cdiv(F, 16)), dim3(256), 0, st, ws, out, (int)nchunk, F, accumulate, scale);
-            OCRL_CHECK_LAUNCH("colsum_final");
-            return 0;
+            return ColsumPlan{true, (R + rpc - 1) / rpc, rpc};
         }
     }
     const int cb = cdiv(F, 64);
@@ -972,12 +1068,71 @@
     if (nchunk < 1) nchunk = 1;
     if (nchunk > (R + 63) / 64) nchunk = (R + 63) / 64;
     if (nchunk < 1) nchunk = 1;
-    OCRL_REQUIRE((size_t)nchunk * F <= ws_floats, "colsum: workspace too small (%lld x %d)", nchunk, F);
-    const long long rpc = (R + nchunk - 1) / nchunk;
-    hipLaunchKernelGGL(colsum_kernel, dim3(cb, (int)nchunk), dim3(256), 0, st, X, ld, ws, R, F, rpc);
-    OCRL_CHECK_LAUNCH("colsum");
-    hipLaunchKernelGGL(colsum_final_kernel, dim3(cdiv(F, 16)), dim3(256), 0, st, ws, out, (int)nchunk, F, accumulate, scale);
+    if ((size_t)nchunk * F > ws_floats) return ColsumPlan{false, 0, 0};
+    return ColsumPlan{false, nchunk, (R + nchunk - 1) / nchunk};
+}
+int colsum_launch(const float* X, long long ld, float* out, long long R, int F, int accumulate, float scale, float* ws, size_t ws_floats, hipStream_t st) {
+    const ColsumPlan pl = colsum_plan(X, ld, R, F, ws_floats);
+    OCRL_REQUIRE(pl.nchunk > 0, "colsum: workspace too small (%lld rows x %d)", R, F);
+    if (pl.vec4) {
+        hipLaunchKernelGGL(colsum4_kernel, dim3((unsigned)pl.nchunk), dim3(256), 0, st, X, ld, ws, R, F, pl.rpc);
+        OCRL_CHECK_LAUNCH("colsum4");
+    } else {
+        hipLaunchKernelGGL(colsum_kernel, dim3(cdiv(F, 64), (int)pl.nchunk), dim3(256), 0, st, X, ld, ws, R, F, pl.rpc);
+        OCRL_CHECK_LAUNCH("colsum");
+    }
+    hipLaunchKernelGGL(colsum_final_kernel, dim3(cdiv(F, 16)), dim3(256), 0, st, ws, out, (int)pl.nchunk, F, accumulate, scale);
     OCRL_CHECK_LAUNCH("colsum_final");
+    return 0;
+}
+int colsum_table_launch(const ColsumSiteHost* sites, int n, hipStream_t st) {
+    OCRL_REQUIRE(n >= 1 && n <= COLSUM_TABLE_MAX, "colsum table: 1 .. %d sites (got %d)", COLSUM_TABLE_MAX, n);
+    ColsumTable t{};
+    long long max4 = 0, max1 = 0;
+    int cb1 = 0, maxF = 0;
+    for (int i = 0; i < n; ++i) {
+        const ColsumSiteHost& h = sites[i];
+        const ColsumPlan pl = colsum_plan(h.X, h.ld, h.R, h.F, h.ws_floats);
+        OCRL_REQUIRE(pl.nchunk > 0, "colsum table: workspace of site %d too small (%lld rows x %d)", i, h.R, h.F);
+        t.s[i] = ColsumSite{h.X, h.ld, h.ws, h.out, h.R, pl.rpc, h.F, (int)pl.nchunk, h.accumulate, pl.vec4 ? 1 : 0};
+        if (pl.vec4) { if (pl.nchunk > max4) max4 = pl.nchunk; }
+        else { if (pl.nchunk > max1) max1 = pl.nchunk; if (cdiv(h.F, 64) > cb1) cb1 = cdiv(h.F, 64); }
+        if (h.F > maxF) maxF = h.F;
+    }
+    if (max4) {
+        hipLaunchKernelGGL(colsum4_table_kernel, dim3((unsigned)max4, n), dim3(256), 0, st, t);
+        OCRL_CHECK_LAUNCH("colsum4_table");
+    }
+    if (max1) {
+        hipLaunchKernelGGL(colsum_table_kernel, dim3(cb1, (unsigned)max1, n), dim3(256), 0, st, t);
+        OCRL_CHECK_LAUNCH("colsum_table");
+    }
+    hipLaunchKernelGGL(colsum_final_table_kernel, dim3(cdiv(maxF, 16), n), dim3(256), 0, st, t);
+    OCRL_CHECK_LAUNCH("colsum_final_table");
+    return 0;
+}
+static int layernorm_bwd_kernels(const float* dy, const float* x, const float* mean, const float* rstd, const float* g, float* dx, float* part,
+                                 long long R, int F, int accumulate_dx, int nblk, const LnBwdTailHost* tail, hipStream_t st) {
+    dim3 grid(nblk), blk(256);
+    const bool tl = tail && (tail->dy2 || tail->drop);
+    const LnBwdTail t = tl ? LnBwdTail{tail->dy2, tail->drop, tail->p, tail->seed, tail->site} : LnBwdTail{nullptr, nullptr, 0.f, 0ull, 0u};
+    const bool al16 = aligned16(x, dy, dx, g, part) && aligned16(t.dy2, t.drop);
+#define LN_BWD(...) do { if (tl) hipLaunchKernelGGL((__VA_ARGS__, true>), grid, blk, 0, st, dy, x, mean, rstd, g, dx, part, R, accumulate_dx, t); \
+                            else hipLaunchKernelGGL((__VA_ARGS__, false>), grid, blk, 0, st, dy, x, mean, rstd, g, dx, part, R, accumulate_dx, t); } while (0)
+    switch (F / 64) {
+        case 1:
+            if (al16) LN_BWD(layernorm16_bwd_kernel<1, 4);
+            else LN_BWD(layernorm_bwd_kernel<1);
+            break;
+        case 2: LN_BWD(layernorm_bwd_kernel<2); break;
+        case 3:
+            if (al16) LN_BWD(layernorm16_bwd_kernel<3, 2);
+            else LN_BWD(layernorm_bwd_kernel<3);
+            break;
+        default: LN_BWD(layernorm_bwd_kernel<4); break;
+    }
+#undef LN_BWD
+    OCRL_CHECK_LAUNCH("layernorm_bwd");
     return 0;
 }
 int layernorm_bwd_launch(const float* dy, const float* x, const float* mean, const float* rstd, const float* g, float* dx,
@@ -988,22 +1143,22 @@
     while (nblk > 64 && (size_t)nblk * 2 * F * 2 + (size_t)8 * 2 * F > ws_floats) nblk /= 2;
     const size_t need = (size_t)nblk * 2 * F;
     OCRL_REQUIRE(need + (size_t)8 * 2 * F <= ws_floats, "layernorm bwd: workspace too small");
-    dim3 grid(nblk), blk(256);
-    const bool al16 = aligned16(x, dy, dx, g, ws);
-    switch (F / 64) {
-        case 1:
-            if (al16) hipLaunchKernelGGL((layernorm16_bwd_kernel<1, 4>), grid, blk, 0, st, dy, x, mean, rstd, g, dx, ws, R, accumulate_dx);
-            else hipLaunchKernelGGL(layernorm_bwd_kernel<1>, grid, blk, 0, st, dy, x, mean, rstd, g, dx, ws, R, accumulate_dx);
-            break;
-        case 2: hipLaunchKernelGGL(layernorm_bwd_kernel<2>, grid, blk, 0, st, dy, x, mean, rstd, g, dx, ws, R, accumulate_dx); break;
-        case 3:
-            if (al16) hipLaunchKernelGGL((layernorm16_bwd_kernel<3, 2>), grid, blk, 0, st, dy, x, mean, rstd, g, dx, ws, R, accumulate_dx);
-            else hipLaunchKernelGGL(layernorm_bwd_kernel<3>, grid, blk, 0, st, dy, x, mean, rstd, g, dx, ws, R, accumulate_dx);
-            break;
-        default: hipLaunchKernelGGL(layernorm_bwd_kernel<4>, grid, blk, 0, st, dy, x, mean, rstd, g, dx, ws, R, accumulate_dx); break;
-    }
-    OCRL_CHECK_LAUNCH("layernorm_bwd");
+    RC(layernorm_bwd_kernels(dy, x, mean, rstd, g, dx, ws, R, F, accumulate_dx, nblk, nullptr, st));
     return colsum_launch(ws, 2 * F, dgb, nblk, 2 * F, accumulate_dgb, 1.f, ws + need, ws_floats - need, st);
+}
+int layernorm_bwd_part_blocks(long long R, int F, size_t part_floats) {
+    int nblk = (int)((R + 3) / 4 < 2048 ? (R + 3) / 4 : 2048);
+    while (nblk > 64 && (size_t)nblk * 2 * F > part_floats) nblk /= 2;
+    return (size_t)nblk * 2 * F <= part_floats ? nblk : 0;
+}
+int layernorm_bwd_part_launch(const float* dy, const float* x, const float* mean, const float* rstd, const float* g, float* dx, long long R, int F,
+                              int accumulate_dx, const LnBwdTailHost& tail, float* part, size_t part_floats, int* nblk_out, hipStream_t st) {
+    OCRL_REQUIRE(F % 64 == 0 && F >= 64 && F <= 256, "layernorm bwd: F must be 64..256, multiple of 64 (got %d)", F);
+    const int nblk = layernorm_bwd_part_blocks(R, F, part_floats);
+    OCRL_REQUIRE(nblk > 0, "layernorm bwd: partial table too small");
+    RC(layernorm_bwd_kernels(dy, x, mean, rstd, g, dx, part, R, F, accumulate_dx, nblk, &tail, st));
+    *nblk_out = nblk;
+    return 0;
 }
 int reduce_partials_launch(const float* part, int n, float* out, float scale, int accumulate, hipStream_t st) {
     hipLaunchKernelGGL(reduce_partials_kernel, dim3(1), dim3(256), 0, st, part, n, out, scale, accumulate);
diff --git a/ocrl_amd/csrc/kernels.h b/ocrl_amd/csrc/kernels.h
--- a/ocrl_amd/csrc/kernels.h
+++ b/ocrl_amd/csrc/kernels.h
@@ -236,6 +236,12 @@
 int layernorm_bwd_launch(const float* dy, const float* x, const float* mean, const float* rstd, const float* g, float* dx,
                          float* dgb, long long R, int F, int accumulate_dx, int accumulate_dgb, float* ws, size_t ws_floats, hipStream_t st);
 int colsum_launch(const float* X, long long ld, float* out, long long R, int F, int accumulate, float scale, float* ws, size_t ws_floats, hipStream_t st);
+struct LnBwdTailHost { const float* dy2 = nullptr; float* drop = nullptr; float p = 0.f; unsigned long long seed = 0; unsigned site = 0; };
+int layernorm_bwd_part_blocks(long long R, int F, size_t part_floats);
+int layernorm_bwd_part_launch(const float* dy, const float* x, const float* mean, const float* rstd, const float* g, float* dx, long long R, int F,
+                              int accumulate_dx, const LnBwdTailHost& tail, float* part, size_t part_floats, int* nblk_out, hipStream_t st);
+struct ColsumSiteHost { const float* X; long long ld; float* out; long long R; int F; int accumulate; float* ws; size_t ws_floats; };
+int colsum_table_launch(const ColsumSiteHost* sites, int n, hipStream_t st);
 
 #define SA_INPUT_SLAB (2 * 4096 + 4 * 64)
 void sa_input_plan(long long R, int max_wgs, int out[3]);
diff --git a/ocrl_amd/csrc/ln_tails_unit.cpp b/ocrl_amd/csrc/ln_tails_unit.cpp
--- /dev/null
+++ b/ocrl_amd/csrc/ln_tails_unit.cpp
@@ -0,0 +1,56 @@
+#include "../../include/ocrl_hip_ln_tails.h"
+#include "common.h"
+#include "kernels.h"
+
+namespace {
+constexpr long long MAX_ELEMS = 0x7fffffffLL;
+constexpr int MAX_SITES = 16;
+int check_ln(const char* who, long long R, int F) {
+    OCRL_REQUIRE(F == 64 || F == 128 || F == 192 || F == 256, "%s: F must be 64, 128, 192 or 256 (got %d)", who, F);
+    OCRL_REQUIRE(R >= 1 && R * F <= MAX_ELEMS, "%s: R >= 1 and R * F < 2^31 (got R %lld)", who, R);
+    return 0;
+}
+}
+
+extern "C" {
+
+int ocrl_lt_site_size(void) { return (int)sizeof(ocrl_lt_site); }
+
+int ocrl_lt_layernorm_bwd_blocks(long long R, int F, size_t part_floats) {
+    if (!(F == 64 || F == 128 || F == 192 || F == 256) || R < 1 || R * F > MAX_ELEMS) return 0;
+    return layernorm_bwd_part_blocks(R, F, part_floats);
+}
+
+int ocrl_lt_layernorm_bwd(const float* dy, const float* dy2, const float* x, const float* mean, const float* rstd, const float* gamma, float* dx,
+                          float* drop, long long R, int F, int accumulate_dx, float p, unsigned long long seed, unsigned site, float* part,
+                          size_t part_floats, int nblk[1], void* stream) {
+    RC(check_ln("ocrl_lt_layernorm_bwd", R, F));
+    OCRL_REQUIRE(dy && x && mean && rstd && gamma && dx && part && nblk, "ocrl_lt_layernorm_bwd: null argument");
+    OCRL_REQUIRE(p >= 0.f && p < 1.f, "ocrl_lt_layernorm_bwd: 0 <= p < 1 (got %g)", (double)p);
+    OCRL_REQUIRE(drop != dx && drop != part, "ocrl_lt_layernorm_bwd: drop must be a buffer of its own");
+    OCRL_REQUIRE(layernorm_bwd_part_blocks(R, F, part_floats) > 0, "ocrl_lt_layernorm_bwd: partial table too small (%zu floats)", part_floats);
+    LnBwdTailHost t;
+    t.dy2 = dy2; t.drop = drop; t.p = p; t.seed = seed; t.site = site;
+    return layernorm_bwd_part_launch(dy, x, mean, rstd, gamma, dx, R, F, accumulate_dx ? 1 : 0, t, part, part_floats, nblk,
+                                     static_cast<hipStream_t>(stream));
+}
+
+int ocrl_lt_colsum_table(const ocrl_lt_site* sites, int n, void* stream) {
+    OCRL_REQUIRE(sites, "ocrl_lt_colsum_table: null argument");
+    OCRL_REQUIRE(n >= 1 && n <= MAX_SITES, "ocrl_lt_colsum_table: 1 <= n <= %d sites (got %d)", MAX_SITES, n);
+    ColsumSiteHost h[MAX_SITES];
+    for (int i = 0; i < n; ++i) {
+        const ocrl_lt_site& s = sites[i];
+        OCRL_REQUIRE(s.X && s.out && s.ws, "ocrl_lt_colsum_table: null argument in site %d", i);
+        OCRL_REQUIRE(s.R >= 1 && s.R <= MAX_ELEMS && s.F >= 1 && s.F <= 65536, "ocrl_lt_colsum_table: site %d: 1 <= R < 2^31 and 1 <= F <= 65536 (got %lld, %d)",
+                     i, s.R, s.F);
+        OCRL_REQUIRE(s.ld >= s.F && s.ld <= MAX_ELEMS, "ocrl_lt_colsum_table: site %d: ld >= F (got ld %lld, F %d)", i, s.ld, s.F);
+        OCRL_REQUIRE(aligned16(s.ws), "ocrl_lt_colsum_table: site %d: ws must be 16-byte aligned", i);
+        for (int j = 0; j < i; ++j)
+            OCRL_REQUIRE(sites[j].out != s.out && sites[j].ws != s.ws, "ocrl_lt_colsum_table: sites %d and %d share out or ws", j, i);
+        h[i] = ColsumSiteHost{s.X, s.ld, s.out, s.R, s.F, s.accumulate ? 1 : 0, s.ws, s.ws_floats};
+    }
+    return colsum_table_launch(h, n, static_cast<hipStream_t>(stream));
+}
+
+}
diff --git a/ocrl_amd/csrc/slate_model.cpp b/ocrl_amd/csrc/slate_model.cpp
--- a/ocrl_amd/csrc/slate_model.cpp
+++ b/ocrl_amd/csrc/slate_model.cpp
@@ -260,6 +260,9 @@
         q.gbr[1] = carve(nullptr, BT * d); q.gbr[2] = carve(nullptr, BT * d);
     }
     scratch3_ = carve(nullptr, scratch_floats_);
+    ln_part_floats_ = (size_t)(BT / 4 < 2048 ? (BT + 3) / 4 : 2048) * 2 * d;
+    ln_sum_floats_ = (size_t)256 * 2 * d;
+    ln_part_ = carve(nullptr, (size_t)(1 + 3 * NB) * (ln_part_floats_ + ln_sum_floats_));
     gmem_ = carve(nullptr, BK * d); gck_ = carve(nullptr, BK * d); gcv_ = carve(nullptr, BK * d);
     gdA_ = carve(nullptr, BN * 64); gdB_ = carve(nullptr, BN * 64);
     }
@@ -698,9 +701,22 @@
     RC(after(W, L, ring_event()));
     RC(lin_bwd_w(pred_, V, lnf_, d, G(w_.out), nullptr, BT, V, d, 1.f, W, ce));
     RC(lin_bwd_x(pred_, V, P(w_.out), gt1_, d, BT, V, d, nullptr, 0, nullptr, 0, L, Drop(), ce));
+    const float* gd = gx_;
+    std::vector<ColsumSiteHost> ln_sites;
+    auto ln_bwd = [&](const float* x, const float* mean, const float* rstd, const float* gamma, float* dgb, int accumulate, const float* dy2,
+                      unsigned drop_site, float* into) -> int {
+        LnBwdTailHost t;
+        t.dy2 = dy2;
+        gd = gx_;
+        if (into && (p > 0.f || dws)) { t.drop = into; t.p = p; t.seed = last_.seed; t.site = drop_site; gd = into; }
+        float* part = ln_part_ + ln_sites.size() * (ln_part_floats_ + ln_sum_floats_);
+        int nblk = 0;
+        RC(layernorm_bwd_part_launch(gt1_, x, mean, rstd, gamma, gx_, BT, d, accumulate, t, part, ln_part_floats_, &nblk, L));
+        ln_sites.push_back(ColsumSiteHost{part, 2 * d, dgb, nblk, 2 * d, 0, part + ln_part_floats_, ln_sum_floats_});
+        return 0;
+    };
     const float* xlast = blk_[NB - 1].x3;
-    RC(layernorm_bwd_launch(gt1_, xlast, lnf_mean_, lnf_rstd_, P(w_.lnf.w), gx_, G(w_.lnf.w), BT, d, 0, 0,
-                            L.scratch, L.scratch_floats, L));
+    RC(ln_bwd(xlast, lnf_mean_, lnf_rstd_, P(w_.lnf.w), G(w_.lnf.w), 0, nullptr, SITE_BLK_BASE + 8 * (NB - 1) + 4, bg_[dws ? NB - 1 : 0].gbr[0]));
     RC(fill_launch(gmem_, BK * d, 0.f, L));
     for (int b = NB - 1; b >= 0; --b) {
         Blk& k = blk_[b];
@@ -708,21 +724,12 @@
         const DecBlockW& bw = w_.blk[b];
         const unsigned site = SITE_BLK_BASE + 8 * b;
         const float* xin = (b == 0) ? emb_ : blk_[b - 1].x3;
-        const float* gd = gx_;
-        auto drop_gx = [&](unsigned s_, float* into) -> int {
-            gd = gx_;
-            if (p > 0.f || dws) { RC(dropout_apply_launch(gx_, into, BT * d, p, last_.seed, s_, L)); gd = into; }
-            return 0;
-        };
-        RC(drop_gx(site + 4, q.gbr[0]));
         RC(lin_bwd_x(gd, d, P(bw.ffn2.w), q.gf1, 4 * d, BT, d, 4 * d, k.f1, 4 * d, nullptr, 0, L));
         RC(after(W, L, ring_event()));
         RC(lin_bwd_w(gd, d, k.f1, 4 * d, G(bw.ffn2.w), G(bw.ffn2.b), BT, d, 4 * d, 1.f, W));
         RC(lin_bwd_w(q.gf1, 4 * d, k.ln3, d, G(bw.ffn0.w), G(bw.ffn0.b), BT, 4 * d, d, 1.f, W));
         RC(lin_bwd_x(q.gf1, 4 * d, P(bw.ffn0.w), gt1_, d, BT, 4 * d, d, nullptr, 0, nullptr, 0, L));
-        RC(layernorm_bwd_launch(gt1_, k.x2, k.ln3_mean, k.ln3_rstd, P(bw.ln3.w), gx_, G(bw.ln3.w), BT, d, 1, 0,
-                                L.scratch, L.scratch_floats, L));
-        RC(drop_gx(site + 3, q.gbr[1]));
+        RC(ln_bwd(k.x2, k.ln3_mean, k.ln3_rstd, P(bw.ln3.w), G(bw.ln3.w), 1, nullptr, site + 3, q.gbr[1]));
         const float* gd_co = gd;
         if (xattn_) {
             XaHost hx = xattn_args(b);
@@ -749,9 +756,7 @@
             RC(lin_bwd_x(gck_, d, P(bw.ck), gmem_, d, BK, d, d, nullptr, 0, gmem_, d, X));
             RC(lin_bwd_x(gcv_, d, P(bw.cv), gmem_, d, BK, d, d, nullptr, 0, gmem_, d, X));
         }
-        RC(layernorm_bwd_launch(gt1_, k.x1, k.ln2_mean, k.ln2_rstd, P(bw.ln2.w), gx_,
-                                G(bw.ln2.w), BT, d, 1, 0, L.scratch, L.scratch_floats, L));
-        RC(drop_gx(site + 1, q.gbr[2]));
+        RC(ln_bwd(k.x1, k.ln2_mean, k.ln2_rstd, P(bw.ln2.w), G(bw.ln2.w), 1, nullptr, site + 1, q.gbr[2]));
         const float* gd_o = gd;
         RC(lin_bwd_x(gd, d, P(bw.o), gt1_, d, BT, d, d, nullptr, 0, nullptr, 0, L));
         {
@@ -765,21 +770,21 @@
         RC(lin_bwd_w(q.gqkv, 3 * d, k.ln1, d, G(bw.qkv), nullptr, BT, 3 * d, d, 1.f, W));
         RC(lin_bwd_x(q.gqkv, 3 * d, P(bw.qkv), gt1_, d, BT, 3 * d, d, nullptr, 0, nullptr, 0, L));
         if (b == 0) {
-            RC(axpy_launch(gx_, gt1_, BT * d, 1.f, L));
-            RC(layernorm_bwd_launch(gt1_, xin, k.ln1_mean, k.ln1_rstd, P(bw.ln1.w), gx_,
-                                    G(bw.ln1.w), BT, d, 0, 0, L.scratch, L.scratch_floats, L));
+            RC(ln_bwd(xin, k.ln1_mean, k.ln1_rstd, P(bw.ln1.w), G(bw.ln1.w), 0, gx_, 0, nullptr));
         } else {
-            RC(layernorm_bwd_launch(gt1_, xin, k.ln1_mean, k.ln1_rstd, P(bw.ln1.w), gx_,
-                                    G(bw.ln1.w), BT, d, 1, 0, L.scratch, L.scratch_floats, L));
-        }
-    }
-    RC(embed_bwd_launch(gx_, tokens_, G(w_.dict), B, T, V, d, p, last_.seed, L.scratch, L.scratch_floats, L));
-    RC(fill_launch(G(w_.pe), (long long)(T + 1) * d, 0.f, L));
-    RC(colsum_launch(gx_, (long long)T * d, G(w_.pe), B, T * d, 0, 1.f, L.scratch, L.scratch_floats, L));
-    RC(copy_launch(G(w_.pe), G(w_.bos), d, L));
+            RC(ln_bwd(xin, k.ln1_mean, k.ln1_rstd, P(bw.ln1.w), G(bw.ln1.w), 1, nullptr, site - 8 + 4, bg_[dws ? b - 1 : 0].gbr[0]));
+        }
+    }
     if (xattn_) RC(after(L, W, ring_event()));
-    RC(lin_bwd_w(gmem_, d, slots_, D, G(w_.slotproj), nullptr, BK, d, D, 1.f, L));
+    RC(after(W, L, ring_event()));
     RC(lin_bwd_x(gmem_, d, P(w_.slotproj), gslots_, D, BK, d, D, nullptr, 0, nullptr, 0, L));
+    for (size_t i = 0; i < ln_sites.size(); i += 16)
+        RC(colsum_table_launch(ln_sites.data() + i, (int)(ln_sites.size() - i < 16 ? ln_sites.size() - i : 16), W));
+    RC(embed_bwd_launch(gx_, tokens_, G(w_.dict), B, T, V, d, p, last_.seed, W.scratch, W.scratch_floats, W));
+    RC(fill_launch(G(w_.pe), (long long)(T + 1) * d, 0.f, W));
+    RC(colsum_launch(gx_, (long long)T * d, G(w_.pe), B, T * d, 0, 1.f, W.scratch, W.scratch_floats, W));
+    RC(copy_launch(G(w_.pe), G(w_.bos), d, W));
+    RC(lin_bwd_w(gmem_, d, slots_, D, G(w_.slotproj), nullptr, BK, d, D, 1.f, W));
     return 0;
 }
 
diff --git a/ocrl_amd/csrc/slate_model.h b/ocrl_amd/csrc/slate_model.h
--- a/ocrl_amd/csrc/slate_model.h
+++ b/ocrl_amd/csrc/slate_model.h
@@ -180,6 +180,8 @@
     float *gA_, *gB_, *gC_;
     float *gdA_, *gdB_;
     float *gmap_;
+    float* ln_part_ = nullptr;
+    size_t ln_part_floats_ = 0, ln_sum_floats_ = 0;
     float *col0_, *dw0p_;
     float* obs_keep_ = nullptr;
     bool first_direct() const { return cfg.obs_channels == 3; }
```

Result: no change. 1801, median of 6 (+0.5%).
